# Diegotistical/OptionsLab

Hardware: AMD Instinct MI355X
Metric: MC path-steps/sec (1M paths × 252 steps Euro call); price vs BS |err|/σ (higher is better)
Workload: dtype f32 normals / f64 prices

## Files before the change

include/olmc.h:

```cpp
#ifndef OLMC_H
#define OLMC_H

#include <stdint.h>

#ifdef __cplusplus
extern "C" {
#endif

#define OLMC_ABI_VERSION 6

enum {
    OLMC_OK = 0,
    OLMC_ERR_ARG = 1,
    OLMC_ERR_HIP = 2,
    OLMC_ERR_STATE = 3,
    OLMC_ERR_RCCL = 4
};

enum { OLMC_STREAM_GBM = 0, OLMC_STREAM_HESTON = 1, OLMC_STREAM_JUMP = 2, OLMC_STREAM_KOU = 3 };
enum { OLMC_STREAM_HESTON_QE = 0x48514500 };
enum { OLMC_AVG_ARITHMETIC = 0, OLMC_AVG_GEOMETRIC = 1, OLMC_AVG_ARITHMETIC_FAST = 2 };
#define OLMC_MAX_BATCH 16

typedef struct olmc_stats {
// ... 139 lines not shown
                      const uint32_t* sv, const uint32_t* shift, int32_t bits, olmc_stats* out);
int olmc_european_qmc_cv(double S, double K, double T, double r, double sigma, double q, int is_call,
                         int64_t point_offset, int64_t n_paths, int32_t dims,
                         const uint32_t* sv, const uint32_t* shift, int32_t bits, olmc_cv_moments* out);

int olmc_european_qmc_batch(const olmc_option* opts, int32_t k, int64_t point_offset, int64_t n_paths, int32_t dims,
                            const uint32_t* sv, const uint32_t* shift, int32_t bits, olmc_stats* out );
int olmc_european_qmc_greeks_fd(double S, double K, double T, double r, double sigma, double q, int is_call,
                                int64_t n_paths, int32_t dims, const uint32_t* sv, const uint32_t* shift, int32_t bits,
                                int second_order, double* out9, olmc_stats* evals );

int olmc_european_qmc_terminal(double S, double T, double r, double sigma, double q,
                               int64_t point_offset, int64_t n_paths, int32_t dims,
                               const uint32_t* sv, const uint32_t* shift, int32_t bits,
                               int antithetic, double* out_host );

enum { OLMC_QMC_SEQUENTIAL = 0, OLMC_QMC_BRIDGE = 1 };
#define OLMC_QMC_BRIDGE_MAX_STEPS 1024
int olmc_asian_qmc(double S, double K, double T, double r, double sigma, double q, int is_call, int avg_kind, int construction,
                   int64_t point_offset, int64_t n_points, int32_t n_steps, const uint32_t* sv, const uint32_t* shift, int32_t bits,
                   int antithetic, olmc_stats* out);
int olmc_extrema_qmc(double S, double K, double T, double r, double sigma, double q, int is_call, int payoff, double barrier,
                     int construction, int64_t point_offset, int64_t n_points, int32_t n_steps, const uint32_t* sv,
                     const uint32_t* shift, int32_t bits, int antithetic, olmc_stats* out);
int olmc_asian_qmc_greeks_fd(double S, double K, double T, double r, double sigma, double q, int is_call, int avg_kind,
                             int construction, int64_t n_points, int32_t n_steps, const uint32_t* sv, const uint32_t* shift,
                             int32_t bits, int antithetic, int second_order, double* out9, olmc_stats* evals );
int olmc_extrema_qmc_greeks_fd(double S, double K, double T, double r, double sigma, double q, int is_call, int payoff, double barrier,
                               int construction, int64_t n_points, int32_t n_steps, const uint32_t* sv, const uint32_t* shift,
                               int32_t bits, int antithetic, int second_order, double* out9, olmc_stats* evals );

int olmc_autocallable_qmc(double S, double T, double r, double sigma, double q, double autocall_barrier, double coupon_barrier,
                          double coupon_rate, double ki_barrier, int32_t observation_freq, int construction,
                          int64_t point_offset, int64_t n_points, int32_t n_steps, const uint32_t* sv, const uint32_t* shift,
                          int32_t bits, int antithetic, olmc_stats* out);
int olmc_cliquet_qmc(double S, double T, double r, double sigma, double q, double local_cap, double local_floor, double global_cap,
                     double global_floor, int32_t n_periods, int construction, int64_t point_offset, int64_t n_points,
                     int32_t n_steps, const uint32_t* sv, const uint32_t* shift, int32_t bits, int antithetic, olmc_stats* out);

int olmc_american_lsm_qmc(double S, double K, double T, double r, double sigma, double q, int is_call, int construction,
                          int64_t n_points, int32_t n_steps, const uint32_t* sv, const uint32_t* shift, int32_t bits,
                          int32_t poly_degree, olmc_stats* out);
int olmc_exercise_boundary_qmc(double S, double K, double T, double r, double sigma, double q, int is_call, int construction,
                               int64_t n_points, int32_t n_steps, const uint32_t* sv, const uint32_t* shift, int32_t bits,
                               double* boundary_host);
int olmc_gbm_qmc_paths(double S, double T, double r, double sigma, double q, int construction, int64_t n_points, int32_t n_steps,
                       const uint32_t* sv, const uint32_t* shift, int32_t bits, int path_major, double* out_host);

int olmc_heston_qmc(double S, double K, double T, double r, double q, int is_call, double kappa, double theta, double sigma_v,
                    double rho, double v0, int construction, int64_t point_offset, int64_t n_points, int32_t n_steps,
                    const uint32_t* sv, const uint32_t* shift, int32_t bits, int antithetic, olmc_stats* out);
int olmc_heston_qmc_paths(double S, double T, double r, double q, double kappa, double theta, double sigma_v, double rho, double v0,
                          int construction, int64_t n_points, int32_t n_steps, const uint32_t* sv, const uint32_t* shift,
                          int32_t bits, int path_major, double* spot_host, double* var_host);

enum { OLMC_PATH_ASIAN_ARITHMETIC = 6, OLMC_PATH_ASIAN_GEOMETRIC = 7 };
int olmc_heston_path_payoff(double S, double K, double T, double r, double q, int is_call, double kappa, double theta, double sigma_v,
                            double rho, double v0, int payoff, double barrier, int64_t path_offset, int64_t n_local, int32_t n_steps,
                            uint64_t seed, int antithetic, olmc_stats* out);
int olmc_heston_qmc_path_payoff(double S, double K, double T, double r, double q, int is_call, double kappa, double theta, double sigma_v,
                                double rho, double v0, int payoff, double barrier, int construction, int64_t point_offset,
                                int64_t n_points, int32_t n_steps, const uint32_t* sv, const uint32_t* shift, int32_t bits,
                                int antithetic, olmc_stats* out);

int olmc_heston_surface(double S, double T, double r, double q, int is_call, double kappa, double theta, double sigma_v, double rho,
                        double v0, const double* strikes, const int32_t* steps, int32_t k, int64_t path_offset, int64_t n_local,
                        int32_t n_steps, uint64_t seed, int antithetic, olmc_stats* out );
int olmc_heston_qmc_surface(double S, double T, double r, double q, int is_call, double kappa, double theta, double sigma_v, double rho,
                            double v0, const double* strikes, const int32_t* steps, int32_t k, int construction, int64_t point_offset,
                            int64_t n_points, int32_t n_steps, const uint32_t* sv, const uint32_t* shift, int32_t bits, int antithetic,
                            olmc_stats* out );

typedef struct olmc_heston_scenario {
    double  S, K, T, r, q, kappa, theta, sigma_v, rho, v0;
    int32_t is_call;
    int32_t pad;
} olmc_heston_scenario;
#define OLMC_HESTON_MAX_RECURSIONS 6
int olmc_heston_scenario_layout(const olmc_heston_scenario* sc, int32_t k, int32_t* n_recursions, int32_t* group );
int olmc_heston_scenarios(const olmc_heston_scenario* sc, int32_t k, int64_t path_offset, int64_t n_local, int32_t n_steps, uint64_t seed,
                          int antithetic, olmc_stats* out );
int olmc_heston_qmc_scenarios(const olmc_heston_scenario* sc, int32_t k, int construction, int64_t point_offset, int64_t n_points,
                              int32_t n_steps, const uint32_t* sv, const uint32_t* shift, int32_t bits, int antithetic,
                              olmc_stats* out );
int olmc_heston_greeks_fd(double S, double K, double T, double r, double sigma, double q, int is_call, double kappa, double theta,
                          double sigma_v, double rho, int64_t n_paths, int32_t n_steps, uint64_t seed, int antithetic, int second_order,
                          double* out9, olmc_stats* evals );
int olmc_heston_qmc_greeks_fd(double S, double K, double T, double r, double sigma, double q, int is_call, double kappa, double theta,
                              double sigma_v, double rho, int construction, int64_t n_points, int32_t n_steps, const uint32_t* sv,
                              const uint32_t* shift, int32_t bits, int antithetic, int second_order, double* out9,
                              olmc_stats* evals );

int olmc_heston_qe_surface(double S, double T, double r, double q, int is_call, double kappa, double theta, double sigma_v, double rho,
                           double v0, const double* strikes, const int32_t* steps, int32_t k, int64_t path_offset, int64_t n_local,
                           int32_t n_steps, uint64_t seed, int antithetic, olmc_stats* out );
int olmc_heston_qe_qmc_surface(double S, double T, double r, double q, int is_call, double kappa, double theta, double sigma_v, double rho,
                               double v0, const double* strikes, const int32_t* steps, int32_t k, int construction, int64_t point_offset,
                               int64_t n_points, int32_t n_steps, const uint32_t* sv, const uint32_t* shift, int32_t bits, int antithetic,
                               olmc_stats* out );
int olmc_heston_qe_paths(double S, double T, double r, double q, double kappa, double theta, double sigma_v, double rho, double v0,
                         int64_t n_paths, int32_t n_steps, uint64_t seed, int path_major, double* spot_host, double* var_host);
int olmc_heston_qe_qmc_paths(double S, double T, double r, double q, double kappa, double theta, double sigma_v, double rho, double v0,
                             int construction, int64_t n_points, int32_t n_steps, const uint32_t* sv, const uint32_t* shift, int32_t bits,
                             int path_major, double* spot_host, double* var_host);

enum { OLMC_HESTON_EULER = 0, OLMC_HESTON_QE = 1 };
int olmc_heston_autocallable(double S, double T, double r, double q, double kappa, double theta, double sigma_v, double rho, double v0,
                             double autocall_barrier, double coupon_barrier, double coupon_rate, double ki_barrier, int32_t observation_freq,
                             int scheme, int64_t path_offset, int64_t n_local, int32_t n_steps, uint64_t seed, int antithetic,
                             olmc_stats* out);
int olmc_heston_autocallable_qmc(double S, double T, double r, double q, double kappa, double theta, double sigma_v, double rho, double v0,
                                 double autocall_barrier, double coupon_barrier, double coupon_rate, double ki_barrier,
                                 int32_t observation_freq, int scheme, int construction, int64_t point_offset, int64_t n_points,
                                 int32_t n_steps, const uint32_t* sv, const uint32_t* shift, int32_t bits, int antithetic, olmc_stats* out);
int olmc_heston_cliquet(double S, double T, double r, double q, double kappa, double theta, double sigma_v, double rho, double v0,
                        double local_cap, double local_floor, double global_cap, double global_floor, int32_t n_periods, int scheme,
                        int64_t path_offset, int64_t n_local, int32_t n_steps, uint64_t seed, int antithetic, olmc_stats* out);
int olmc_heston_cliquet_qmc(double S, double T, double r, double q, double kappa, double theta, double sigma_v, double rho, double v0,
                            double local_cap, double local_floor, double global_cap, double global_floor, int32_t n_periods, int scheme,
                            int construction, int64_t point_offset, int64_t n_points, int32_t n_steps, const uint32_t* sv,
                            const uint32_t* shift, int32_t bits, int antithetic, olmc_stats* out);

int olmc_multi_gpu_european(double S, double K, double T, double r, double sigma, double q, int is_call,
                            int64_t n_paths, int32_t n_steps, uint64_t seed, int antithetic,
                            int n_gpus, olmc_stats* out);
int olmc_multi_gpu_greeks_fd(double S, double K, double T, double r, double sigma, double q, int is_call,
                             int64_t n_paths, int32_t n_steps, uint64_t seed, int second_order,
                             int n_gpus, double* out9, olmc_stats* evals );
int olmc_multi_gpu_european_cv(double S, double K, double T, double r, double sigma, double q, int is_call,
                               int64_t n_paths, int32_t n_steps, uint64_t seed, int antithetic,
                               int n_gpus, olmc_cv_moments* out);
int olmc_multi_gpu_european_qmc(double S, double K, double T, double r, double sigma, double q, int is_call,
                                int64_t n_paths, int32_t dims, const uint32_t* sv, const uint32_t* shift, int32_t bits,
                                int n_gpus, olmc_stats* out);
int olmc_multi_gpu_european_qmc_greeks_fd(double S, double K, double T, double r, double sigma, double q, int is_call,
                                          int64_t n_paths, int32_t dims, const uint32_t* sv, const uint32_t* shift, int32_t bits,
                                          int second_order, int n_gpus, double* out9, olmc_stats* evals );
int olmc_multi_gpu_european_qmc_cv(double S, double K, double T, double r, double sigma, double q, int is_call,
                                   int64_t n_paths, int32_t dims, const uint32_t* sv, const uint32_t* shift, int32_t bits,
                                   int n_gpus, olmc_cv_moments* out);
int olmc_multi_gpu_spans(double* out8);

int olmc_fetch_dev(const double* d_src, int32_t n, void* hip_stream, double* out_host);

int olmc_combine_stats(const olmc_stats* parts, int32_t n_parts, double r, double T, olmc_stats* out);

int olmc_philox_words(uint64_t seed, int64_t path_offset, int64_t n_paths,
                      int32_t block0, int32_t n_blocks, uint32_t stream_tag, uint32_t* out_host);
int olmc_normals(uint64_t seed, int64_t path_offset, int64_t n_paths, int32_t n_steps,
                 float* out_host);

int olmc_profile_enable(int on);
enum { OLMC_TUNE_GRID_CAP = 2, OLMC_TUNE_QMC_BLOCK = 4, OLMC_TUNE_SPLIT_TAIL = 7, OLMC_TUNE_POLL = 8, OLMC_TUNE_SPLIT_SAT = 9,
       OLMC_TUNE_MULTI_LAUNCH = 10, OLMC_TUNE_STAGED_COPY = 11, OLMC_TUNE_PHILOX_TABLE = 12 };
int olmc_tune(int knob, int value);
int olmc_profile_reset(void);
int olmc_kernel_time(int64_t* launches, double* total_ms);

#ifdef __cplusplus
}
#endif
#endif
```

optionslab_amd/_hip.py:

```python
from __future__ import annotations

import ctypes as C
import importlib.util
import os
import sys
import threading
from typing import List, Optional, Sequence, Tuple

import numpy as np

from .exceptions import AccelerationError

LIBRARY_PATH = os.environ.get("OLMC_LIBRARY") or os.path.join(os.path.dirname(os.path.abspath(__file__)), "libolmc.so")
MAX_BATCH = 16
AVG_ARITHMETIC, AVG_GEOMETRIC, AVG_ARITHMETIC_FAST = 0, 1, 2
_U64 = (1 << 64) - 1


class Stats(C.Structure):
    _fields_ = [("sum", C.c_double), ("sumsq", C.c_double), ("n", C.c_int64),
                ("price", C.c_double), ("std_error", C.c_double)]


class Option(C.Structure):
# ... 864 lines not shown


def heston_qe_qmc_surface(S, T, r, q, is_call: bool, kappa, theta, sigma_v, rho, v0, strikes, steps, n_points: int, sv: np.ndarray,
                          shift: np.ndarray, bridge: bool = False, antithetic: bool = False, point_offset: int = 0) -> List[Stats]:
    sobol = _sobol_args(sv, shift, point_offset, n_points, 2)
    cells = _SurfaceCells(strikes, steps)
    return cells.answer(lib().olmc_heston_qe_qmc_surface(S, T, r, q, int(is_call), kappa, theta, sigma_v, rho, v0, *cells.run, _construction(bridge),
                                                         int(point_offset), int(n_points), *sobol.run, int(antithetic), cells.out))


HESTON_EULER, HESTON_QE = 0, 1


def _scheme(qe: bool) -> int:
    return HESTON_QE if qe else HESTON_EULER


def heston_autocallable(S, T, r, q, kappa, theta, sigma_v, rho, v0, autocall_barrier, coupon_barrier, coupon_rate, ki_barrier,
                        observation_freq: int, n_paths: int, n_steps: int, seed: int, antithetic: bool = False, path_offset: int = 0,
                        qe: bool = False) -> Stats:
    return _answer(lib().olmc_heston_autocallable(S, T, r, q, kappa, theta, sigma_v, rho, v0, autocall_barrier, coupon_barrier, coupon_rate, ki_barrier,
                                                  int(observation_freq), _scheme(qe), int(path_offset), int(n_paths), int(n_steps),
                                                  seed64(seed), int(antithetic), _byref(out := Stats())), out)


def heston_autocallable_qmc(S, T, r, q, kappa, theta, sigma_v, rho, v0, autocall_barrier, coupon_barrier, coupon_rate, ki_barrier,
                            observation_freq: int, n_points: int, sv: np.ndarray, shift: np.ndarray, bridge: bool = True,
                            antithetic: bool = False, point_offset: int = 0, qe: bool = False) -> Stats:
    sobol = _sobol_args(sv, shift, point_offset, n_points, 2)
    return _answer(lib().olmc_heston_autocallable_qmc(S, T, r, q, kappa, theta, sigma_v, rho, v0, autocall_barrier, coupon_barrier, coupon_rate, ki_barrier,
                                                      int(observation_freq), _scheme(qe), _construction(bridge), int(point_offset), int(n_points),
                                                      *sobol.run, int(antithetic), _byref(out := Stats())), out)


def heston_cliquet(S, T, r, q, kappa, theta, sigma_v, rho, v0, local_cap, local_floor, global_cap, global_floor, n_periods: int,
                   n_paths: int, n_steps: int, seed: int, antithetic: bool = False, path_offset: int = 0, qe: bool = False) -> Stats:
    return _answer(lib().olmc_heston_cliquet(S, T, r, q, kappa, theta, sigma_v, rho, v0, local_cap, local_floor, global_cap, global_floor, int(n_periods),
                                             _scheme(qe), int(path_offset), int(n_paths), int(n_steps),
                                             seed64(seed), int(antithetic), _byref(out := Stats())), out)


def heston_cliquet_qmc(S, T, r, q, kappa, theta, sigma_v, rho, v0, local_cap, local_floor, global_cap, global_floor, n_periods: int,
                       n_points: int, sv: np.ndarray, shift: np.ndarray, bridge: bool = True, antithetic: bool = False,
                       point_offset: int = 0, qe: bool = False) -> Stats:
    sobol = _sobol_args(sv, shift, point_offset, n_points, 2)
    return _answer(lib().olmc_heston_cliquet_qmc(S, T, r, q, kappa, theta, sigma_v, rho, v0, local_cap, local_floor, global_cap, global_floor, int(n_periods),
                                                 _scheme(qe), _construction(bridge), int(point_offset), int(n_points),
                                                 *sobol.run, int(antithetic), _byref(out := Stats())), out)


def heston_qe_paths(S, T, r, q, kappa, theta, sigma_v, rho, v0, n_paths: int, n_steps: int, seed: int, path_major: bool = False):
    return _spot_and_variance(lib().olmc_heston_qe_paths, n_paths, n_steps, path_major, S, T, r, q, kappa, theta, sigma_v, rho, v0,
                              int(n_paths), int(n_steps), seed64(seed))


def heston_qe_qmc_paths(S, T, r, q, kappa, theta, sigma_v, rho, v0, n_points: int, sv: np.ndarray, shift: np.ndarray, bridge: bool = False,
                        path_major: bool = False):
    sobol = _sobol_args(sv, shift, 0, n_points, 2)
    return _spot_and_variance(lib().olmc_heston_qe_qmc_paths, n_points, sobol.steps, path_major, S, T, r, q, kappa, theta, sigma_v, rho, v0,
                              _construction(bridge), int(n_points), *sobol.run)


def _basis(spot_basis: bool) -> int:
    return HA_BASIS_SPOT if spot_basis else HA_BASIS_SPOT_VARIANCE


def heston_american_lsm(S, K, T, r, q, is_call: bool, kappa, theta, sigma_v, rho, v0, n_paths: int, n_steps: int, seed: int, poly_degree: int = 2,
                        spot_basis: bool = False, qe: bool = False) -> Stats:
    return _answer(lib().olha_american_lsm(S, K, T, r, q, int(is_call), kappa, theta, sigma_v, rho, v0, _scheme(qe), _basis(spot_basis), int(poly_degree),
                                           int(n_paths), int(n_steps), seed64(seed), _byref(out := Stats())), out)


def heston_american_lsm_qmc(S, K, T, r, q, is_call: bool, kappa, theta, sigma_v, rho, v0, n_points: int, sv: np.ndarray, shift: np.ndarray,
                            bridge: bool = True, poly_degree: int = 2, spot_basis: bool = False, qe: bool = False) -> Stats:
    steps, psv, psh, bits = _sobol_args(sv, shift, 0, n_points, 2).run
    return _answer(lib().olha_american_lsm_qmc(S, K, T, r, q, int(is_call), kappa, theta, sigma_v, rho, v0, _scheme(qe), _basis(spot_basis), int(poly_degree),
                                               _construction(bridge), int(n_points), psv, psh, 2 * steps, bits, _byref(out := Stats())), out)


def heston_american_scales(S, K, T, r, q, is_call: bool, kappa, theta, sigma_v, v0, n_steps: int):
    out = [np.empty(int(n_steps) + 1 if n_steps >= 1 else 1, dtype=np.float64) for _ in range(4)]
    _check(load_library().olha_regressor_scales(S, K, T, r, q, int(is_call), kappa, theta, sigma_v, v0, int(n_steps), *[_dp(a) for a in out]))
    return tuple(out)


def multi_gpu_european(S, K, T, r, sigma, q, is_call: bool, n_paths: int, n_steps: int, seed: int, antithetic: bool,
                       n_gpus: int) -> Stats:
    return _answer(lib().olmc_multi_gpu_european(S, K, T, r, sigma, q, int(is_call), int(n_paths), int(n_steps), seed64(seed),
                                                 int(antithetic), int(n_gpus), _byref(out := Stats())), out)


def multi_gpu_greeks_fd(S, K, T, r, sigma, q, is_call: bool, n_paths: int, n_steps: int, seed: int, second_order: bool, n_gpus: int,
                        want_evals: bool = True) -> Tuple[List[float], List[Stats]]:
    return _greeks(want_evals, lib().olmc_multi_gpu_greeks_fd, S, K, T, r, sigma, q, int(is_call), int(n_paths), int(n_steps), seed64(seed),
                   int(second_order), int(n_gpus))


def multi_gpu_european_cv(S, K, T, r, sigma, q, is_call: bool, n_paths: int, n_steps: int, seed: int, antithetic: bool, n_gpus: int) -> CvMoments:
    return _answer(lib().olmc_multi_gpu_european_cv(S, K, T, r, sigma, q, int(is_call), int(n_paths), int(n_steps), seed64(seed),
                                                    int(antithetic), int(n_gpus), _byref(out := CvMoments())), out)


def multi_gpu_european_qmc(S, K, T, r, sigma, q, is_call: bool, n_paths: int, sv: np.ndarray, shift: np.ndarray, n_gpus: int) -> Stats:
    sobol = _sobol_args(sv, shift, 0, n_paths)
    return _answer(lib().olmc_multi_gpu_european_qmc(S, K, T, r, sigma, q, int(is_call), int(n_paths), *sobol.run, int(n_gpus), _byref(out := Stats())), out)


def multi_gpu_european_qmc_greeks_fd(S, K, T, r, sigma, q, is_call: bool, n_paths: int, sv: np.ndarray, shift: np.ndarray, second_order: bool,
                                     n_gpus: int, want_evals: bool = True) -> Tuple[List[float], List[Stats]]:
    sobol = _sobol_args(sv, shift, 0, n_paths)
    return _greeks(want_evals, lib().olmc_multi_gpu_european_qmc_greeks_fd, S, K, T, r, sigma, q, int(is_call), int(n_paths), *sobol.run,
                   int(second_order), int(n_gpus))


def multi_gpu_european_qmc_cv(S, K, T, r, sigma, q, is_call: bool, n_paths: int, sv: np.ndarray, shift: np.ndarray, n_gpus: int) -> CvMoments:
    sobol = _sobol_args(sv, shift, 0, n_paths)
    return _answer(lib().olmc_multi_gpu_european_qmc_cv(S, K, T, r, sigma, q, int(is_call), int(n_paths),
                                                        *sobol.run, int(n_gpus), _byref(out := CvMoments())), out)


def multi_gpu_spans() -> dict:
    out = (C.c_double * 8)()
    _check(lib().olmc_multi_gpu_spans(out))
    return dict(zip(("launch_us", "collective_us", "fetch_us", "drain_us", "total_us", "wake_us_max", "rank_launch_us_max", "rank_launch_us_min"), out))


def combine_stats(parts: Sequence[Tuple[float, float, int]], r: float, T: float) -> Stats:
    k = len(parts)
    arr = (Stats * k)(*[Stats(s, ss, int(n), 0.0, 0.0) for (s, ss, n) in parts])
    return _answer(load_library().olmc_combine_stats(arr, k, r, T, _byref(out := Stats())), out)


def philox_words(seed: int, path_offset: int, n_paths: int, block0: int, n_blocks: int, tag: int = 0) -> np.ndarray:
    out = np.empty((int(n_paths), int(n_blocks), 4), dtype=np.uint32)
    _check(lib().olmc_philox_words(seed64(seed), int(path_offset), int(n_paths), int(block0), int(n_blocks), int(tag),
                                   _pointer(out, C.c_uint32)))
    return out


def normals(seed: int, path_offset: int, n_paths: int, n_steps: int) -> np.ndarray:
    out = np.empty((int(n_paths), int(n_steps)), dtype=np.float32)
    _check(lib().olmc_normals(seed64(seed), int(path_offset), int(n_paths), int(n_steps), _pointer(out, C.c_float)))
    return out


TUNE_GRID_CAP = 2
TUNE_QMC_BLOCK = 4
TUNE_SPLIT_TAIL = 7
TUNE_POLL = 8
TUNE_SPLIT_SAT = 9
TUNE_MULTI_LAUNCH = 10
TUNE_STAGED_COPY = 11
TUNE_PHILOX_TABLE = 12


def tune(knob: int, value: int) -> None:
    _check(load_library().olmc_tune(int(knob), int(value)))


def profile_enable(on: bool) -> None:
    _check(lib().olmc_profile_enable(int(on)))


def profile_reset() -> None:
    _check(lib().olmc_profile_reset())


def kernel_time() -> Tuple[int, float]:
    n, ms = C.c_int64(0), C.c_double(0.0)
    _check(lib().olmc_kernel_time(C.byref(n), C.byref(ms)))
    return n.value, ms.value
```

optionslab_amd/csrc/olmc.hip:

```cpp
#include "olmc.h"
#include "olmc_local_vol.h"
#include "olmc_local_vol_qmc.h"
#include "olmc_jump.h"
#include "olha.h"
#include "olmc_kernels.h"
#include "olmc_local_vol_kernels.h"
#include "olmc_local_vol_qmc_kernels.h"
#include "olmc_jump_kernels.h"
#include "olmc_jump_scenario_kernels.h"
#include "olmc_heston_american_kernels.h"
#include "olmc_job_board.h"
#include "olmc_device_mem.h"

#include <dlfcn.h>
#include <sched.h>
#include <time.h>
#include <hip/hip_ext.h>
#include <rccl/rccl.h>

#include <algorithm>
#include <atomic>
#include <chrono>
#include <climits>
#include <condition_variable>
// ... 158 lines not shown
    DevicePool* pool = nullptr;
    CtxLease() = default;
    CtxLease(const CtxLease&) = delete;
    CtxLease& operator=(const CtxLease&) = delete;
    ~CtxLease() { release(); }
    void release() {
        if (!c) return;
        {
            std::lock_guard<std::mutex> lock(pool->mu);
            c->busy = false;
        }
        pool->idle.notify_all();
        c = nullptr;
    }
};

int ctx_lease_on(int dev, CtxLease* out) {
    DevicePool* pool = g_pool[dev].load(std::memory_order_acquire);
    if (!pool) return fail(OLMC_ERR_STATE, "device not initialised (call olmc_init)");
    HIP_TRY(hipSetDevice(dev));
    std::unique_lock<std::mutex> lock(pool->mu);
    for (;;) {
        for (DeviceCtx* c : pool->all)
            if (!c->busy) {
                c->busy = true;
                out->c = c;
                out->pool = pool;
                return OLMC_OK;
            }
        if (static_cast<int>(pool->all.size()) < kMaxContexts) {
            DeviceCtx* c = nullptr;
            const int rc = ctx_create(dev, &c);
            if (rc) return rc;
            c->busy = true;
            pool->all.push_back(c);
            out->c = c;
            out->pool = pool;
            return OLMC_OK;
        }
        pool->idle.wait(lock);
    }
}

int ctx_lease(CtxLease* out) {
    int dev = t_device >= 0 ? t_device : g_default_device.load(std::memory_order_acquire);
    if (dev < 0) {
        int rc = olmc_init(0);
        if (rc) return rc;
        dev = t_device;
    }
    return ctx_lease_on(dev, out);
}

int bulk_reserve(DeviceCtx* c, size_t bytes, Carver* spans = nullptr) {
    const int rc = c->bulk.reserve(bytes, [c] { return c->drain(); });
    if (spans) *spans = c->bulk.carve();
    return rc;
}

constexpr size_t kStageBytes = size_t(16) << 20, kStagedFrom = size_t(32) << 20;
int g_staged_copy = 0;

int copy_to_host(DeviceCtx* c, void* dst, const void* d_src, size_t bytes) {
    if (bytes < kStagedFrom || g_staged_copy < 0) {
        HIP_TRY(hipMemcpyAsync(dst, d_src, bytes, hipMemcpyDeviceToHost, c->stream));
        HIP_TRY(hipStreamSynchronize(c->stream));
        return OLMC_OK;
    }
    for (int i = 0; i < 2; ++i) {
        const int rc = c->stage[i].reserve(kStageBytes, no_users);
        if (rc) return rc;
        if (!c->stage_landed[i]) HIP_TRY(hipEventCreateWithFlags(&c->stage_landed[i], hipEventDisableTiming));
    }
    cpu_set_t cpus;
    int allowed = 4;
    if (sched_getaffinity(0, sizeof cpus, &cpus) == 0) allowed = CPU_COUNT(&cpus);
    const int n_threads = std::max(1, std::min(8, allowed / 2));
    const int64_t n_chunks = static_cast<int64_t>((bytes + kStageBytes - 1) / kStageBytes);
    std::atomic<int64_t> landed{0};
    std::atomic<int> copied[2] = {{0}, {0}};
    std::atomic<bool> give_up{false};
    auto chunk_len = [&](int64_t i) { return std::min(kStageBytes, bytes - static_cast<size_t>(i) * kStageBytes); };
    auto worker = [&](int w) {
        for (int64_t i = 0; i < n_chunks; ++i) {
            for (uint32_t spins = 0; landed.load(std::memory_order_acquire) <= i; ++spins) {
                if (give_up.load(std::memory_order_relaxed)) return;
                if ((spins & 0xFF) == 0xFF) sched_yield(); else __builtin_ia32_pause();
            }
            const size_t len = chunk_len(i), per = (len / n_threads + 4095) & ~size_t(4095);
            const size_t lo = std::min(len, per * w), hi = std::min(len, lo + per);
            if (hi > lo) std::memcpy(static_cast<char*>(dst) + static_cast<size_t>(i) * kStageBytes + lo, static_cast<const char*>(c->stage[i & 1].get()) + lo, hi - lo);
            copied[i & 1].fetch_add(1, std::memory_order_release);
        }
    };
    static const bool trace = std::getenv("OLMC_TRACE_COPY") != nullptr;
    using clock = std::chrono::steady_clock;
    auto us_since = [](clock::time_point t) { return std::chrono::duration<double, std::micro>(clock::now() - t).count(); };
    const auto t_begin = clock::now();
    double us_spawn = 0, us_first = 0, us_events = 0, us_workers = 0;
    std::vector<std::thread> threads;
    threads.reserve(n_threads);
    try {
        for (int w = 0; w < n_threads; ++w) threads.emplace_back(worker, w);
    } catch (const std::system_error&) {
        give_up.store(true);
        for (std::thread& t : threads) t.join();
        HIP_TRY(hipMemcpyAsync(dst, d_src, bytes, hipMemcpyDeviceToHost, c->stream));
        HIP_TRY(hipStreamSynchronize(c->stream));
        return OLMC_OK;
    }
    us_spawn = us_since(t_begin);
    hipError_t err = hipSuccess;
    for (int64_t i = 0; i < n_chunks && err == hipSuccess; ++i) {
        const int slot = static_cast<int>(i & 1);
        if (i >= 2) {
            const auto t = clock::now();
            for (uint32_t spins = 0; copied[slot].load(std::memory_order_acquire) < n_threads; ++spins)
                if ((spins & 0xFF) == 0xFF) sched_yield(); else __builtin_ia32_pause();
            copied[slot].store(0, std::memory_order_relaxed);
            us_workers += us_since(t);
        }
        err = hipMemcpyAsync(c->stage[slot].get(), static_cast<const char*>(d_src) + static_cast<size_t>(i) * kStageBytes, chunk_len(i), hipMemcpyDeviceToHost, c->stream);
        if (err == hipSuccess) err = hipEventRecord(c->stage_landed[slot], c->stream);
        if (err == hipSuccess && i >= 1) {
            const auto t = clock::now();
            err = hipEventSynchronize(c->stage_landed[slot ^ 1]);
            if (i == 1) us_first = us_since(t); else us_events += us_since(t);
            if (err == hipSuccess) landed.store(i, std::memory_order_release);
        }
    }
    {
        const auto t = clock::now();
        if (err == hipSuccess) err = hipEventSynchronize(c->stage_landed[(n_chunks - 1) & 1]);
        us_events += us_since(t);
    }
    if (err == hipSuccess) landed.store(n_chunks, std::memory_order_release);
    else give_up.store(true);
    const auto t_join = clock::now();
    for (std::thread& t : threads) t.join();
    if (trace)
        std::fprintf(stderr, "[olmc copy_to_host] %.1f MB, %lld chunks, %d threads: spawn %.0f us, first chunk landed (kernel + DMA) %.0f us, later event waits %.0f us, "
                             "waits for the copy threads %.0f us, last chunk out + join %.0f us, total %.0f us\n", bytes / 1e6, static_cast<long long>(n_chunks), n_threads,
                     us_spawn, us_first, us_events, us_workers, us_since(t_join), us_since(t_begin));
    if (err != hipSuccess) {
        (void)hipStreamSynchronize(c->stream);
        (void)hipGetLastError();
        return fail(OLMC_ERR_HIP, std::string("copy_to_host: ") + hipGetErrorString(err));
    }
    return OLMC_OK;
}

int g_multi_launch = 0;
int g_grid_cap = 0;
int g_qmc_block = 0;
int g_poll = 0;
int g_split_tail = 0;
int g_philox_table = 1;
int g_split_sat = 0;
#ifdef OLMC_WITH_PROBES
int g_fault_shard = 0;
int g_force_nv = 0;
int g_multi_rehearsal = 0;
int g_expect_table = 0;
std::atomic<int> g_expect_table_misses{0};
#endif

int32_t grid_for(int64_t n_paths, int32_t n_steps = INT32_MAX) { return path_grid(n_paths, n_steps, g_grid_cap); }

template <typename Kernel>
int resident_workgroups(Kernel kernel) {
    static std::mutex mu;
    static std::vector<std::pair<const void*, int>> cache;
    const void* key = reinterpret_cast<const void*>(kernel);
    std::lock_guard<std::mutex> lock(mu);
    for (const auto& e : cache)
        if (e.first == key) return e.second;
    int nb = 0;
    if (hipOccupancyMaxActiveBlocksPerMultiprocessor(&nb, kernel, kBlock, 0) != hipSuccess || nb < 1) {
        (void)hipGetLastError();
        nb = 1;
    }
    cache.emplace_back(key, nb);
    return nb;
}

int32_t european_launch_shape(const DeviceCtx* c, PathRange* pr, int occ, bool keep_grid = false) {
    pr->split_from = INT32_MAX;
    const int grid_cap = keep_grid ? 0 : g_grid_cap;
    const int32_t grid = path_grid(pr->count, pr->n_steps, grid_cap);
    const int64_t wgs = (pr->count + kBlock - 1) / kBlock;
    if (g_split_tail < 0 || grid_cap != 0 || wgs != grid) return grid;
    if ((pr->n_steps >> 2) / kGroup < 4 || c->cus < 1) return grid;
    int64_t per_cu = (pr->count / kBlock) / c->cus;
    if (occ >= 1 && g_split_sat > 0) {
        const int64_t r = per_cu % occ;
        if (r > 0 && r < std::min(g_split_sat, occ)) per_cu -= r;
    }
    const int64_t full = per_cu * c->cus;
    const int64_t rest = pr->count - full * kBlock;
    if (rest == 0) return grid;
    const int64_t split = (rest + kWave - 1) / kWave;
    if (full + split > kMaxGrid) return grid;
    pr->split_from = static_cast<int32_t>(full);
    return static_cast<int32_t>(full + split);
}

template <int NSETS, int MODE>
int european_occupancy(bool anti) {
    if (g_split_sat <= 0) return 0;
    return anti ? resident_workgroups(european_path_kernel<NSETS, true, MODE, false>) : resident_workgroups(european_path_kernel<NSETS, false, MODE, false>);
}

int make_ws(DeviceCtx* c, hipStream_t stream, int32_t grid, int nv, double* d_out, double tail, ReduceWs* ws) {
    const bool own = stream == c->stream;
    int idx = DeviceCtx::kSlots;
    if (!own) {
        idx = -1;
        for (int i = 0; i < DeviceCtx::kSlots && idx < 0; ++i)
            if (c->slots[i].claimed && !c->slots[i].shared && c->slots[i].owner == stream) idx = i;
        for (int i = 0; i < DeviceCtx::kSlots && idx < 0; ++i)
            if (!c->slots[i].claimed) { c->slots[i].claimed = true; c->slots[i].owner = stream; idx = i; }
        if (idx < 0) {
            idx = c->next_slot;
            c->next_slot = (c->next_slot + 1) % DeviceCtx::kSlots;
            DeviceCtx::WsSlot& taken = c->slots[idx];
            if (!taken.shared) {
                HIP_TRY(hipDeviceSynchronize());
                taken.shared = true;
                taken.used = false;
            }
        }
    }
    DeviceCtx::WsSlot& sl = c->slots[idx];
    c->cur_slot = idx;
    const bool guarded = !own && sl.shared;
    const size_t need = static_cast<size_t>(grid) * nv;
    int rc = sl.block_rows.reserve(sizeof(double) * need, [&] {
        if (!guarded) HIP_TRY(hipStreamSynchronize(stream));
        else if (sl.used) HIP_TRY(hipEventSynchronize(sl.done));
        return static_cast<int>(OLMC_OK);
    }, sizeof(double) << 16);
    if (rc) return rc;
    if (guarded && sl.used) HIP_TRY(hipStreamWaitEvent(stream, sl.done, 0));
    ws->block_rows = sl.block_rows.as<double>();
    ws->group_rows = sl.group_rows.as<double>();
    ws->counters = sl.counters.as<uint32_t>();
    ws->out = d_out;
    ws->tail = tail;
    ws->row_capacity = sl.block_rows.capacity() / sizeof(double);
#ifdef OLMC_WITH_PROBES
    if (g_force_nv > 0) ws->row_capacity = static_cast<uint64_t>(grid) * g_force_nv;
#endif
    ws->done_flag = nullptr;
    ws->done_value = 0;
    c->armed = 0;
    if (own && d_out == c->d_result && g_poll >= 0) {
        c->armed = ++c->seq;
        ws->done_flag = c->d_flag;
        ws->done_value = c->armed;
    }
    return OLMC_OK;
}

void ws_recover(DeviceCtx* c) {
    c->armed = 0;
    (void)hipDeviceSynchronize();
    (void)hipGetLastError();
    for (auto& sl : c->slots) (void)hipMemset(sl.counters.get(), 0, kCounterBytes);
}

void multi_recover(DeviceCtx* c) {
    c->armed = 0;
    (void)hipDeviceSynchronize();
    (void)hipGetLastError();
    if (c->multi.counters()) (void)hipMemset(c->multi.counters(), 0, c->multi.counter_bytes());
}

int after_launch(DeviceCtx* c, hipStream_t stream) {
    hipError_t e = hipGetLastError();
    if (e != hipSuccess) { ws_recover(c); return fail(OLMC_ERR_HIP, std::string("kernel launch: ") + hipGetErrorString(e)); }
    if (c->cur_slot == DeviceCtx::kSlots || !c->slots[c->cur_slot].shared) return OLMC_OK;
    DeviceCtx::WsSlot& sl = c->slots[c->cur_slot];
    HIP_TRY(hipEventRecord(sl.done, stream));
    sl.used = true;
    return OLMC_OK;
}

int prof_begin(DeviceCtx* c, hipStream_t s, EventPair* ep) {
    if (c->ev_free.empty()) {
        HIP_TRY(hipEventCreate(&ep->start));
        HIP_TRY(hipEventCreate(&ep->stop));
    } else {
        *ep = c->ev_free.back();
        c->ev_free.pop_back();
    }
    HIP_TRY(hipEventRecord(ep->start, s));
    return OLMC_OK;
}

int prof_acquire(DeviceCtx* c, EventPair* ep) {
    if (c->ev_free.empty()) {
        HIP_TRY(hipEventCreate(&ep->start));
        HIP_TRY(hipEventCreate(&ep->stop));
    } else {
        *ep = c->ev_free.back();
        c->ev_free.pop_back();
    }
    return OLMC_OK;
}

int prof_end(DeviceCtx* c, hipStream_t s, const EventPair& ep) {
    HIP_TRY(hipEventRecord(ep.stop, s));
    c->ev_pending.push_back(ep);
    return OLMC_OK;
}

int prof_drain(DeviceCtx* c) {
    for (const EventPair& ep : c->ev_pending) {
        float ms = 0.f;
        if (hipEventSynchronize(ep.stop) == hipSuccess && hipEventElapsedTime(&ms, ep.start, ep.stop) == hipSuccess) {
            c->prof_ms += ms;
            c->prof_launches += 1;
        } else {
            (void)hipGetLastError();
        }
        c->ev_free.push_back(ep);
    }
    c->ev_pending.clear();
    return OLMC_OK;
}


int check_paths(int64_t path_offset, int64_t n_local, int32_t n_steps) {
    if (n_local < 1) return fail(OLMC_ERR_ARG, "n_paths must be >= 1");
    if (n_steps < 1) return fail(OLMC_ERR_ARG, "n_steps must be >= 1");
    if (path_offset < 0) return fail(OLMC_ERR_ARG, "path_offset must be >= 0");
    return OLMC_OK;
}

PathRange make_range(int64_t path_offset, int64_t n_local, int32_t n_steps, uint64_t seed) {
    PathRange pr;
    pr.first = static_cast<uint64_t>(path_offset);
    pr.count = n_local;
    pr.n_steps = n_steps;
    pr.key0 = static_cast<uint32_t>(seed);
    pr.key1 = static_cast<uint32_t>(seed >> 32);
    pr.split_from = INT32_MAX;
    return pr;
}

template <typename Kernel, typename... Args>
void launch_timed(Kernel kernel, dim3 grid, dim3 block, hipStream_t s, const EventPair* timed, const Args&... args) {
    if (timed) hipExtLaunchKernelGGL(kernel, grid, block, 0, s, timed->start, timed->stop, 0, args...);
    else hipLaunchKernelGGL(kernel, grid, block, 0, s, args...);
}

template <typename F>
void with_bool(bool b, F&& f) {
    if (b) f(std::true_type{});
    else f(std::false_type{});
}

template <typename F>
void with_set_anti(int nsets, bool anti, F&& f) {
    with_bool(nsets == 8, [&](auto eight) { with_bool(anti, [&](auto a) { f(std::integral_constant<int, eight ? 8 : 16>{}, a); }); });
}

int prof_pair(DeviceCtx* c, EventPair* ep, const EventPair** timed) {
    *timed = nullptr;
    if (!g_profile) return OLMC_OK;
    int rc = prof_acquire(c, ep);
    if (rc) return rc;
    c->ev_pending.push_back(*ep);
    *timed = ep;
    return OLMC_OK;
}

PhiloxPrefix european_prefix(const PathRange& pr, bool strided) {
    PhiloxPrefix pp;
    const int32_t blocks = (pr.n_steps + 3) / 4;
    const uint64_t last = pr.first + static_cast<uint64_t>(pr.count) - 1;
    const bool table = g_philox_table != 0 && !strided && blocks <= kPrefixBlocks && (last >> 32) == (pr.first >> 32);
    philox_prefix(static_cast<uint64_t>(pr.key0) | static_cast<uint64_t>(pr.key1) << 32, static_cast<uint32_t>(pr.first >> 32), 0u, table ? blocks : 0, &pp);
    return pp;
}

template <int NSETS, int MODE>
void launch_european(bool anti, int32_t grid, hipStream_t s, const PathRange& pr, const ContractSet<NSETS>& cs,
                     const ReduceWs& ws, double* terminal, const EventPair* timed = nullptr) {
    const bool strided = static_cast<int64_t>(grid) * kBlock < pr.count;
    const PhiloxPrefix pp = european_prefix(pr, strided);
#ifdef OLMC_WITH_PROBES
    if (g_expect_table != 0 && (g_expect_table > 0) != (pp.n_blocks != 0)) g_expect_table_misses.fetch_add(1, std::memory_order_relaxed);
#endif
    auto launch = [&](auto strided_c, auto a) {
        launch_timed(european_path_kernel<NSETS, a, MODE, strided_c>, dim3(grid), dim3(kBlock), s, timed, pr, cs, ws, terminal, pp);
    };
    if constexpr (MODE == kSumOnly) with_bool(anti, [&](auto a) { launch(std::false_type{}, a); });
    else with_bool(strided, [&](auto strided_c) { with_bool(anti, [&](auto a) { launch(strided_c, a); }); });
}

int sync_or_recover(DeviceCtx* c, hipStream_t s);

template <typename Launch>
int launch_reduce(DeviceCtx* c, hipStream_t s, double* d_out, double tail, int nv, int32_t grid, Launch&& launch, bool profiled = true) {
    ReduceWs ws;
    int rc = make_ws(c, s, grid, nv, d_out, tail, &ws);
    if (rc) return rc;
    EventPair ep{};
    const EventPair* timed = nullptr;
    if (profiled) {
        rc = prof_pair(c, &ep, &timed);
        if (rc) return rc;
    }
    launch(grid, s, timed, ws);
    rc = after_launch(c, s);
    if (rc || d_out != c->d_result) return rc;
    return sync_or_recover(c, s);
}

void finish_one(const double* h, int64_t n, double r_disc, double T, bool bad, olmc_stats* out) {
    if (bad) nan_stats(n, out);
    else finish_stats(h[0], h[1], n, r_disc, T, out);
}

void finish_set(const double* h, const int* pos, int64_t n, const olmc_option* opts, int64_t k, bool extra_bad, bool lean, olmc_stats* st) {
    for (int64_t i = 0; i < k; ++i) {
        const int64_t slot = pos ? pos[i] : i;
        const olmc_option& o = opts[i];
        if (extra_bad || poisoned(o.S, o.K, o.T, o.r, o.sigma, o.q)) nan_stats(n, &st[i]);
        else if (lean) finish_stats(h[slot], std::nan(""), n, o.r, o.T, &st[i]);
        else finish_stats(h[2 * slot], h[2 * slot + 1], n, o.r, o.T, &st[i]);
    }
}

struct GbmStep {
    double dt, drift, vol;
};
GbmStep gbm_step(double T, int32_t n_steps, double r, double q, double sigma) {
    const double dt = T / n_steps;
    return {dt, (r - q - 0.5 * sigma * sigma) * dt, sigma * std::sqrt(dt)};
}

int run_batch_device(DeviceCtx* c, hipStream_t s, const olmc_option* opts, int32_t k, int64_t path_offset,
                     int64_t n_local, int32_t n_steps, uint64_t seed, int antithetic, double* d_out, double tail,
                     int* pos , bool profiled, bool* sums_only = nullptr
                     ,
                     bool keep_grid = false ) {
    PathRange pr = make_range(path_offset, n_local, n_steps, seed);
    const bool anti = antithetic != 0;
    const int nsets = k == 1 ? 1 : (k <= 8 ? 8 : 16);
    const int occ = nsets == 1 ? european_occupancy<1, kReduce>(anti) : (nsets == 8 ? european_occupancy<8, kReduce>(anti) : european_occupancy<16, kReduce>(anti));
    const int32_t grid = european_launch_shape(c, &pr, occ, keep_grid);
    const bool lean = sums_only && *sums_only && nsets > 1 && static_cast<int64_t>(grid) * kBlock >= n_local;
    if (sums_only) *sums_only = lean;
    return launch_reduce(c, s, d_out, tail, lean ? nsets : 2 * nsets, grid, [&](int32_t g, hipStream_t st, const EventPair* timed, const ReduceWs& ws) {
        auto fused = [&](auto width) {
            ContractSet<width> cs;
            group_contracts<width>(opts, k, n_steps, &cs, pos);
            if (!lean) launch_european<width, kReduce>(anti, g, st, pr, cs, ws, nullptr, timed);
            else launch_european<width, kSumOnly>(anti, g, st, pr, cs, ws, nullptr, timed);
        };
        if (nsets == 1) {
            ContractSet<1> cs;
            cs.c[0] = make_contract(opts[0], n_steps);
            cs.base_mask = 1u; cs.upper_continues_slot0 = 0;
            if (pos) pos[0] = 0;
            launch_european<1, kReduce>(anti, g, st, pr, cs, ws, nullptr, timed);
        } else if (nsets == 8) {
            fused(std::integral_constant<int, 8>{});
        } else {
            fused(std::integral_constant<int, 16>{});
        }
    }, profiled);
}

constexpr int64_t kSpinUs = 200, kYieldUs = 2000, kSleepUs = 20;

struct TimerSlack {
    long old = -1;
    void tighten() {
        if (old >= 0) return;
        old = prctl(PR_GET_TIMERSLACK, 0, 0, 0, 0);
        if (old >= 0 && prctl(PR_SET_TIMERSLACK, 1000UL, 0, 0, 0) != 0) old = -1;
    }
    ~TimerSlack() {
        if (old >= 0) (void)prctl(PR_SET_TIMERSLACK, static_cast<unsigned long>(old), 0, 0, 0);
    }
};

int wait_armed(DeviceCtx* c, hipStream_t s) {
    if (c->armed != 0) {
        const uint64_t want = c->armed;
        c->armed = 0;
        using clock = std::chrono::steady_clock;
        const auto t0 = clock::now();
        bool queried = false;
        int phase = 0;
        TimerSlack slack;
        for (uint32_t spins = 0;; ++spins) {
            if (__atomic_load_n(c->h_flag, __ATOMIC_ACQUIRE) == want) {
                if (queried) (void)hipGetLastError();
                return OLMC_OK;
            }
            if (phase == 0) {
                __builtin_ia32_pause();
                if ((spins & 0x3F) == 0x3F && clock::now() - t0 >= std::chrono::microseconds(kSpinUs)) phase = 1;
// ... 890 lines not shown
    CtxLease lease;
    rc = matrix_prologue(n_paths, n_steps, 2 * bytes, "path matrices would exceed 64 GB", &lease);
    if (rc) return rc;
    DeviceCtx* const c = lease.c;
    const auto hc = Scheme::make(S, T, r, q, 1, m, n_steps);
    const PathRange pr = make_range(0, n_paths, n_steps, seed);
    return heston_path_matrices(c, n_paths, n_steps, spot_host, var_host, [&](const EventPair* timed, double* d_spot, double* d_var) {
        with_bool(path_major != 0, [&](auto pm) {
            launch_timed(Scheme::template paths_kernel<decltype(pm)::value>(), dim3(grid_for(n_paths)), dim3(kBlock), c->stream, timed, pr, hc, S, d_spot,
                         d_var);
        });
    });
}
}

extern "C" int olmc_heston_paths(double S, double T, double r, double q, double kappa, double theta, double sigma_v, double rho,
                                 double v0, int64_t n_paths, int32_t n_steps, uint64_t seed, int path_major, double* spot_host,
                                 double* var_host) {
    return run_heston_paths<HestonEuler>(S, T, r, q, {kappa, theta, sigma_v, rho, v0}, n_paths, n_steps, seed, path_major, spot_host, var_host);
}

extern "C" int olmc_heston(double S, double K, double T, double r, double q, int is_call, double kappa, double theta,
                           double sigma_v, double rho, double v0, int64_t path_offset, int64_t n_local, int32_t n_steps,
                           uint64_t seed, int antithetic, olmc_stats* out) {
    if (!out) return fail(OLMC_ERR_ARG, "null pointer");
    const HestonModel m{kappa, theta, sigma_v, rho, v0};
    const int rc = heston_check(m);
    if (rc) return rc;
    const HestonContract hc = make_heston(S, K, T, r, q, is_call, m, n_steps);
    const bool bad = heston_poisoned(S, K, T, r, q, m);
    return run_structured(path_offset, n_local, n_steps, seed, antithetic, r, T, bad, out,
                          [&](int32_t grid, hipStream_t st, const EventPair* timed, const PathRange& pr, const ReduceWs& ws) {
                              with_bool(antithetic != 0, [&](auto a) { launch_timed(heston_kernel<a>, dim3(grid), dim3(kBlock), st, timed, pr, hc, ws); });
                          });
}

namespace {
int make_jump(double S, double K, double T, double r, double sigma, double q, int is_call, int model, double lambda_j,
              double a1, double a2, double a3, int32_t n_steps, JumpContract* out) {
    if (model != OLMC_JUMP_MERTON && model != OLMC_JUMP_KOU) return fail(OLMC_ERR_ARG, "bad jump model");
    if (!(lambda_j >= 0.0)) return fail(OLMC_ERR_ARG, "lambda_j must be non-negative");
    if (n_steps < 1) return fail(OLMC_ERR_ARG, "n_steps must be >= 1");
    JumpContract jc;
    const double dt = T / n_steps;
    double kappa;
    if (model == OLMC_JUMP_MERTON) {
        jc.mu_j = a1; jc.sigma_j = a2;
        jc.kou_p = 0.0; jc.inv_eta1 = 0.0; jc.inv_eta2 = 0.0;
        kappa = std::exp(a1 + 0.5 * a2 * a2) - 1;
    } else {
        jc.mu_j = 0.0; jc.sigma_j = 0.0;
        jc.kou_p = a1; jc.inv_eta1 = 1.0 / a2; jc.inv_eta2 = 1.0 / a3;
        kappa = a1 * a2 / (a2 - 1) + (1 - a1) * a3 / (a3 + 1) - 1;
    }
    jc.kou = model == OLMC_JUMP_KOU;
    jc.pad = 0;
    jc.log_s0 = std::log(S);
    jc.drift = (r - q - lambda_j * kappa - 0.5 * sigma * sigma) * dt;
    jc.vol = sigma * std::sqrt(dt);
    jc.strike = K;
    jc.sign = is_call ? 1.0 : -1.0;
    jc.lam_dt = lambda_j * dt;
    if (jc.lam_dt > 20.0) return fail(OLMC_ERR_ARG, "lambda_j * T / n_steps must be <= 20 jumps per step: raise n_steps");
    jc.p0 = std::exp(-jc.lam_dt);
    *out = jc;
    return OLMC_OK;
}
}

extern "C" int olmc_jump_diffusion(double S, double K, double T, double r, double sigma, double q, int is_call, int model,
                                   double lambda_j, double a1, double a2, double a3, int64_t path_offset, int64_t n_local,
                                   int32_t n_steps, uint64_t seed, olmc_stats* out) {
    JumpContract jc;
    int rc = make_jump(S, K, T, r, sigma, q, is_call, model, lambda_j, a1, a2, a3, n_steps, &jc);
    if (rc) return rc;
    const bool bad = poisoned(S, K, T, r, sigma, q) || std::isnan(lambda_j + a1 + a2 + a3);
    return run_structured(path_offset, n_local, n_steps, seed, 0, r, T, bad, out,
                          [&](int32_t grid, hipStream_t st, const EventPair* timed, const PathRange& pr, const ReduceWs& ws) {
                              launch_timed(jump_kernel, dim3(grid), dim3(kBlock), st, timed, pr, jc, ws);
                          });
}

extern "C" int olmc_jump_paths(double S, double T, double r, double sigma, double q, int model, double lambda_j, double a1,
                               double a2, double a3, int64_t n_paths, int32_t n_steps, uint64_t seed, int path_major,
                               double* out_host) {
    if (!out_host) return fail(OLMC_ERR_ARG, "null pointer");
    JumpContract jc;
    const int rc = make_jump(S, 0.0, T, r, sigma, q, 1, model, lambda_j, a1, a2, a3, n_steps, &jc);
    if (rc) return rc;
    return run_philox_matrix(n_paths, n_steps, seed, out_host, no_setup,
                             [&](DeviceCtx* c, int32_t grid, const PathRange& pr, double* d_paths) {
        with_bool(path_major != 0, [&](auto pm) {
            launch_timed(jump_paths_kernel<pm>, dim3(grid), dim3(kBlock), c->stream, nullptr, pr, jc, S, d_paths);
        });
    });
}

namespace {
struct SobolArgs {
    int construction;
    int64_t point_offset, n_points;
    int32_t n_steps;
    const uint32_t* sv;
    const uint32_t* shift;
    int32_t bits;
    int antithetic;
};

class SobolCall {
public:
    const bool bridge;
    const int64_t first, count;
    const int32_t n_steps, dims_per_step;
    const uint32_t* const sv;
    const uint32_t* const shift;
    const int32_t bits;
    const bool anti;

    static std::optional<SobolCall> make(const SobolArgs& a, int32_t dims_per_step, int* rc) {
        *rc = check(a, dims_per_step);
        if (*rc) return std::nullopt;
        return SobolCall(a.construction == OLMC_QMC_BRIDGE, a.point_offset, a.n_points, a.n_steps, dims_per_step, a.sv, a.shift, a.bits, a.antithetic != 0);
    }
    SobolCall over(int64_t lo, int64_t n) const { return SobolCall(bridge, lo, n, n_steps, dims_per_step, sv, shift, bits, anti); }

    int32_t dims() const { return n_steps * dims_per_step; }
    int64_t samples() const { return count * (anti ? 2 : 1); }
    QmcRange range() const { return QmcRange{static_cast<uint64_t>(first), count, n_steps, anti ? 1 : 0}; }

private:
    SobolCall(bool bridge_, int64_t first_, int64_t count_, int32_t n_steps_, int32_t dims_per_step_, const uint32_t* sv_, const uint32_t* shift_,
              int32_t bits_, bool anti_)
        : bridge(bridge_), first(first_), count(count_), n_steps(n_steps_), dims_per_step(dims_per_step_), sv(sv_), shift(shift_), bits(bits_),
          anti(anti_) {}

    static int check(const SobolArgs& a, int32_t dims_per_step) {
        if (a.construction != OLMC_QMC_SEQUENTIAL && a.construction != OLMC_QMC_BRIDGE) return fail(OLMC_ERR_ARG, "bad construction");
        if (a.construction == OLMC_QMC_BRIDGE && a.n_steps > OLMC_QMC_BRIDGE_MAX_STEPS)
            return fail(OLMC_ERR_ARG, "the Brownian-bridge construction takes at most OLMC_QMC_BRIDGE_MAX_STEPS (1024) dates");
        static_assert(OLMC_QMC_BRIDGE_MAX_STEPS == kQmcBridgeMaxSteps, "the header's cap is the kernel's LDS size");
        if (dims_per_step == 2 && (a.n_steps < 1 || a.n_steps > 10600))
            return fail(OLMC_ERR_ARG, "n_steps must be in [1, 10600]: a step takes two of the 21201 Sobol dimensions");
        const int32_t dims = a.n_steps * dims_per_step;
        if (!a.sv || !a.shift) return fail(OLMC_ERR_ARG, "null pointer");
        if (a.bits != kSobolBits) return fail(OLMC_ERR_ARG, "only 30-bit Sobol tables (SciPy's default) are supported");
        if (dims < 1 || dims > 21201) return fail(OLMC_ERR_ARG, "dims must be in [1, 21201]");
        const int rc = check_paths(a.point_offset, a.n_points, dims);
        if (rc) return rc;
        if (a.point_offset + a.n_points > (int64_t(1) << kSobolBits)) return fail(OLMC_ERR_ARG, "at most 2**30 Sobol points");
        return OLMC_OK;
    }
};

int qmc_table(DeviceCtx* c, const SobolCall& q, const uint32_t** d_sv, const uint32_t** d_shift) {
    const size_t sv_words = static_cast<size_t>(q.dims()) * kSobolBits;
    const int rc = c->sobol.put(q.sv, sizeof(uint32_t) * sv_words, q.shift, sizeof(uint32_t) * q.dims(), c->stream, [c] { return c->drain(); });
    if (rc) return rc;
    *d_sv = c->sobol.device<uint32_t>();
    *d_shift = *d_sv + sv_words;
    return OLMC_OK;
}

QmcShape qmc_shape(const SobolCall& q) {
    return qmc_launch_shape(q.first, q.count, q.dims(), g_qmc_block, g_grid_cap);
}

template <int MODE>
void launch_qmc_european(const QmcShape& sh, int32_t grid, hipStream_t s, const EventPair* timed, const QmcRange& qr, const Contract& ct,
                         const uint32_t* d_sv, const uint32_t* d_shift, const ReduceWs& ws, double* terminal) {
    auto go = [&](auto kernel) { launch_timed(kernel, dim3(grid), dim3(kBlock), s, timed, qr, ct, d_sv, d_shift, ws, terminal); };
    if (sh.blocks && sh.aligned8) go(european_qmc_block_kernel<MODE, true>);
    else if (sh.blocks) go(european_qmc_block_kernel<MODE, false>);
    else if (sh.split && sh.aligned) go(european_qmc_kernel<MODE, true, true>);
    else if (sh.split) go(european_qmc_kernel<MODE, true, false>);
    else go(european_qmc_kernel<MODE, false, false>);
}

template <int NSETS>
void launch_qmc_batch(const QmcShape& sh, int32_t grid, hipStream_t s, const EventPair* timed, const QmcRange& qr, const ContractSet<NSETS>& cs,
                      const uint32_t* d_sv, const uint32_t* d_shift, const ReduceWs& ws) {
    auto go = [&](auto kernel) { launch_timed(kernel, dim3(grid), dim3(kBlock), s, timed, qr, cs, d_sv, d_shift, ws); };
    if (sh.blocks && sh.aligned8) go(european_qmc_batch_kernel<NSETS, true, false, true>);
    else if (sh.blocks) go(european_qmc_batch_kernel<NSETS, true, false>);
    else if (sh.split && sh.aligned) go(european_qmc_batch_kernel<NSETS, false, true, true>);
    else if (sh.split) go(european_qmc_batch_kernel<NSETS, false, true>);
    else go(european_qmc_batch_kernel<NSETS, false, false>);
}

Contract qmc_contract(double S, double K, double T, double r, double sigma, double q, int is_call, int32_t dims, bool mirror) {
    const GbmStep g = gbm_step(T, dims, r, q, sigma);
    Contract ct;
    ct.vol = g.vol;
    ct.a = mirror ? std::log(S) + (r - q - 0.5 * sigma * sigma) * T : std::log(S) + g.drift * dims;
    ct.strike = K;
    ct.sign = is_call ? 1.0 : -1.0;
    ct.scale = 1.0;
    ct.neg_sign_strike = -ct.sign * K;
    ct.sign_scale = ct.sign;
    return ct;
}

int qmc_device(DeviceCtx* c, const Contract& ct, const SobolCall& q, bool five, double* d_out, double tail, bool profiled) {
    const uint32_t *d_sv, *d_shift;
    int rc = qmc_table(c, q, &d_sv, &d_shift);
    if (rc) return rc;
    const QmcRange qr = q.range();
    const QmcShape sh = qmc_shape(q);
    return launch_reduce(c, c->stream, d_out, tail, five ? 5 : 2, sh.grid, [&](int32_t grid, hipStream_t s, const EventPair* timed, const ReduceWs& ws) {
        if (five) launch_qmc_european<kControlVariate>(sh, grid, s, timed, qr, ct, d_sv, d_shift, ws, nullptr);
        else launch_qmc_european<kReduce>(sh, grid, s, timed, qr, ct, d_sv, d_shift, ws, nullptr);
    }, profiled);
}

int run_qmc(const olmc_option& o, const SobolCall& q, olmc_stats* out, double* terminal_host, olmc_cv_moments* cv = nullptr) {
    CtxLease lease;
    int rc = ctx_lease(&lease);
    if (rc) return rc;
    DeviceCtx* const c = lease.c;
    const Contract ct = qmc_contract(o.S, o.K, o.T, o.r, o.sigma, o.q, o.is_call, q.dims(), q.anti);
    if (!terminal_host) {
        rc = qmc_device(c, ct, q, cv != nullptr, c->d_result, -1.0, true);
        if (rc) return rc;
        if (cv) {
            cv_from_device(c->h_result, q.count, o.S, o.T, o.r, o.q, cv);
            if (poisoned(o.S, o.K, o.T, o.r, o.sigma, o.q)) cv->value = std::nan("");
            return OLMC_OK;
        }
        finish_one(c->h_result, q.count, o.r, o.T, poisoned(o.S, o.K, o.T, o.r, o.sigma, o.q), out);
        return OLMC_OK;
    }
    const size_t term_bytes = sizeof(double) * static_cast<size_t>(q.samples());
    Carver bulk;
    rc = bulk_reserve(c, term_bytes, &bulk);
    if (rc) return rc;
    const uint32_t *d_sv, *d_shift;
    rc = qmc_table(c, q, &d_sv, &d_shift);
    if (rc) return rc;
    double* d_term = bulk.take<double>(term_bytes / sizeof(double));
    const QmcShape sh = qmc_shape(q);
    launch_qmc_european<kTerminal>(sh, sh.grid, c->stream, nullptr, q.range(), ct, d_sv, d_shift, ReduceWs{}, d_term);
    HIP_TRY(hipGetLastError());
    c->armed = 0;
    return copy_to_host(c, terminal_host, d_term, term_bytes);
}

int run_qmc_checked(const olmc_option& o, const SobolArgs& a, olmc_stats* out, double* terminal_host, olmc_cv_moments* cv = nullptr) {
    int rc;
    const auto q = SobolCall::make(a, 1, &rc);
    return q ? run_qmc(o, *q, out, terminal_host, cv) : rc;
}
}

extern "C" int olmc_european_qmc_cv(double S, double K, double T, double r, double sigma, double q, int is_call,
                                    int64_t point_offset, int64_t n_paths, int32_t dims, const uint32_t* sv,
                                    const uint32_t* shift, int32_t bits, olmc_cv_moments* out) {
    if (!out) return fail(OLMC_ERR_ARG, "null pointer");
    return run_qmc_checked(make_option(S, K, T, r, sigma, q, is_call), {OLMC_QMC_SEQUENTIAL, point_offset, n_paths, dims, sv, shift, bits, 0}, nullptr,
                           nullptr, out);
}

extern "C" int olmc_european_qmc(double S, double K, double T, double r, double sigma, double q, int is_call,
                                 int64_t point_offset, int64_t n_paths, int32_t dims, const uint32_t* sv,
                                 const uint32_t* shift, int32_t bits, olmc_stats* out) {
    if (!out) return fail(OLMC_ERR_ARG, "null pointer");
    return run_qmc_checked(make_option(S, K, T, r, sigma, q, is_call), {OLMC_QMC_SEQUENTIAL, point_offset, n_paths, dims, sv, shift, bits, 0}, out,
                           nullptr);
}

extern "C" int olmc_european_qmc_terminal(double S, double T, double r, double sigma, double q, int64_t point_offset,
                                          int64_t n_paths, int32_t dims, const uint32_t* sv, const uint32_t* shift,
                                          int32_t bits, int antithetic, double* out_host) {
    if (!out_host) return fail(OLMC_ERR_ARG, "null pointer");
    return run_qmc_checked(make_option(S, 0.0, T, r, sigma, q, 1), {OLMC_QMC_SEQUENTIAL, point_offset, n_paths, dims, sv, shift, bits, antithetic},
                           nullptr, out_host);
}

namespace {
int qmc_bridge_plan(DeviceCtx* c, int32_t n, QmcBridgePlan* plan) {
    const size_t ab_bytes = (sizeof(uint32_t) * static_cast<size_t>(n) + 7) & ~size_t(7), bytes = ab_bytes + sizeof(double) * 3 * n;
    const int rc = c->bridge.ensure(n, bytes, c->stream, [c] { return c->drain(); }, [&](unsigned char* host) {
        uint32_t* ab = reinterpret_cast<uint32_t*>(host);
        double* coef = reinterpret_cast<double*>(host + ab_bytes);
        std::vector<std::pair<int32_t, int32_t>> queue{{0, n}};
        int32_t k = 1;
        for (size_t head = 0; head < queue.size(); ++head) {
            const int32_t a = queue[head].first, b = queue[head].second;
            if (b - a < 2) continue;
            const int32_t m = (a + b) / 2;
            if (k >= n) return fail(OLMC_ERR_ARG, "bridge plan overflow");
            ab[k] = static_cast<uint32_t>(a) | (static_cast<uint32_t>(b) << 16);
            coef[k] = static_cast<double>(b - m) / (b - a);
            coef[n + k] = static_cast<double>(m - a) / (b - a);
            coef[2 * n + k] = std::sqrt(static_cast<double>((m - a) * (b - m)) / (b - a));
            ++k;
            queue.emplace_back(a, m);
            queue.emplace_back(m, b);
        }
        if (k != n) return fail(OLMC_ERR_ARG, "bridge plan is incomplete");
        return static_cast<int>(OLMC_OK);
    });
    if (rc) return rc;
    plan->ab = c->bridge.device<uint32_t>();
    plan->coef = reinterpret_cast<const double*>(c->bridge.device<unsigned char>() + ab_bytes);
    return OLMC_OK;
}

struct QmcPathLaunch {
    const uint32_t* d_sv;
    const uint32_t* d_shift;
    QmcBridgePlan plan;
    QmcRange qr;
    int32_t grid;
    bool bridge, anti;
    double inv_steps;
    double* slabs = nullptr;
};
int qmc_path_setup(DeviceCtx* c, const SobolCall& q, QmcPathLaunch* pl) {
    int rc = qmc_table(c, q, &pl->d_sv, &pl->d_shift);
    if (rc) return rc;
    pl->plan = QmcBridgePlan{nullptr, nullptr};
    pl->bridge = q.bridge;
    if (pl->bridge) {
        rc = qmc_bridge_plan(c, q.n_steps, &pl->plan);
        if (rc) return rc;
    }
    pl->qr = q.range();
    pl->grid = qmc_point_grid(q.count, g_grid_cap);
    pl->anti = q.anti;
    pl->inv_steps = 1.0 / q.n_steps;
    return OLMC_OK;
}

template <typename F>
void with_bridge_anti(const QmcPathLaunch& pl, F&& f) {
    with_bool(pl.bridge, [&](auto b) { with_bool(pl.anti, [&](auto a) { f(b, a); }); });
}

template <typename F>
void with_qmc_path_family(int family, F&& f) {
    if (family == kQmcAsianArithmetic) f(std::integral_constant<int, kQmcAsianArithmetic>{});
    else if (family == kQmcAsianGeometric) f(std::integral_constant<int, kQmcAsianGeometric>{});
    else f(std::integral_constant<int, kQmcExtrema>{});
}

template <typename Shape, typename Launch, typename Finish>
int run_qmc_reduce(const SobolCall& q, int nv, Shape shape, Launch launch, Finish finish) {
    CtxLease lease;
    int rc = ctx_lease(&lease);
    if (rc) return rc;
    DeviceCtx* const c = lease.c;
    QmcPathLaunch pl;
    rc = qmc_path_setup(c, q, &pl);
    if (rc) return rc;
    rc = shape(c, q, &pl);
    if (rc) return rc;
    rc = launch_reduce(c, c->stream, c->d_result, -1.0, nv, pl.grid,
                       [&](int32_t g, hipStream_t s, const EventPair* timed, const ReduceWs& ws) { launch(g, s, timed, pl, ws); });
    if (rc) return rc;
    finish(c->h_result, q.samples());
    return OLMC_OK;
}
inline int qmc_point_shape(DeviceCtx*, const SobolCall&, QmcPathLaunch*) { return OLMC_OK; }
auto qmc_stats(double r_for_discount, double T, bool poisoned_inputs, olmc_stats* out) {
    return [=](const double* h, int64_t n) { finish_one(h, n, r_for_discount, T, poisoned_inputs, out); };
}

int run_qmc_path(int family, int payoff, const olmc_option& o, double barrier, const SobolArgs& args, olmc_stats* out) {
    if (!out) return fail(OLMC_ERR_ARG, "null pointer");
    int rc;
    const auto q = SobolCall::make(args, 1, &rc);
    if (!q) return rc;
    const ExtremaContract ec = make_extrema(o.S, o.K, o.T, o.r, o.sigma, o.q, o.is_call, family == kQmcExtrema ? payoff : 0, barrier, q->n_steps);
    const bool bad = poisoned(o.S, o.K, o.T, o.r, o.sigma, o.q) || std::isnan(barrier);
    return run_qmc_reduce(*q, 2, qmc_point_shape, [&](int32_t g, hipStream_t s, const EventPair* timed, const QmcPathLaunch& pl, const ReduceWs& ws) {
        with_qmc_path_family(family, [&](auto f) {
            with_bridge_anti(pl, [&](auto b, auto a) {
                launch_timed(qmc_path_kernel<f, b, a>, dim3(g), dim3(kBlock), s, timed, pl.qr, ec, pl.inv_steps, pl.d_sv, pl.d_shift, pl.plan, ws);
            });
        });
    }, qmc_stats(o.r, o.T, bad, out));
}

int run_qmc_path_greeks(int family, int payoff, const olmc_option& o, double barrier, const SobolArgs& args, int second_order, double* out9,
                        olmc_stats* evals) {
    if (!out9) return fail(OLMC_ERR_ARG, "null pointer");
    if (!(o.T > 0.0)) return fail(OLMC_ERR_ARG, "T must be > 0");
    int rc;
    const auto q = SobolCall::make(args, 1, &rc);
    if (!q) return rc;
    const GreeksSet gs(o.S, o.K, o.T, o.r, o.sigma, o.q, o.is_call, second_order);
    ExtremaGreeksSet es;
    if (const char* bad = extrema_greeks_layout(gs, q->n_steps, payoff, barrier, o.K, o.is_call, &es, 1.0)) return fail(OLMC_ERR_STATE, bad);
    const int nsets = gs.nsets();
    return run_qmc_reduce(*q, 2 * nsets, qmc_point_shape, [&](int32_t g, hipStream_t s, const EventPair* timed, const QmcPathLaunch& pl, const ReduceWs& ws) {
        with_qmc_path_family(family, [&](auto f) {
            with_bool(pl.bridge, [&](auto b) {
                with_set_anti(nsets, pl.anti, [&](auto width, auto a) {
                    launch_timed(qmc_path_greeks_kernel<f, b, a, width>, dim3(g), dim3(kBlock), s, timed, pl.qr, es, pl.inv_steps, pl.d_sv, pl.d_shift,
                                 pl.plan, ws);
                });
            });
        });
    }, [&](const double* h, int64_t n) {
        olmc_stats st[OLMC_MAX_BATCH];
        finish_set(h, nullptr, n, gs.o, gs.k, false, false, st);
        gs.finish(st, o.T, out9, evals);
    });
}
}

extern "C" int olmc_asian_qmc(double S, double K, double T, double r, double sigma, double q, int is_call, int avg_kind, int construction,
                              int64_t point_offset, int64_t n_points, int32_t n_steps, const uint32_t* sv, const uint32_t* shift, int32_t bits,
                              int antithetic, olmc_stats* out) {
    if (avg_kind != OLMC_AVG_ARITHMETIC && avg_kind != OLMC_AVG_GEOMETRIC) return fail(OLMC_ERR_ARG, "bad avg_kind (arithmetic or geometric)");
    return run_qmc_path(avg_kind == OLMC_AVG_GEOMETRIC ? kQmcAsianGeometric : kQmcAsianArithmetic, 0, make_option(S, K, T, r, sigma, q, is_call), 0.0,
                        {construction, point_offset, n_points, n_steps, sv, shift, bits, antithetic}, out);
}

extern "C" int olmc_extrema_qmc(double S, double K, double T, double r, double sigma, double q, int is_call, int payoff, double barrier,
                                int construction, int64_t point_offset, int64_t n_points, int32_t n_steps, const uint32_t* sv,
                                const uint32_t* shift, int32_t bits, int antithetic, olmc_stats* out) {
    if (payoff < OLMC_BARRIER_UP_OUT || payoff > OLMC_LOOKBACK_FIXED) return fail(OLMC_ERR_ARG, "bad payoff");
    if (payoff <= OLMC_BARRIER_DOWN_IN && !(barrier > 0.0)) return fail(OLMC_ERR_ARG, "Barrier must be positive");
    return run_qmc_path(kQmcExtrema, payoff, make_option(S, K, T, r, sigma, q, is_call), payoff <= OLMC_BARRIER_DOWN_IN ? barrier : 0.0,
                        {construction, point_offset, n_points, n_steps, sv, shift, bits, antithetic}, out);
}

extern "C" int olmc_asian_qmc_greeks_fd(double S, double K, double T, double r, double sigma, double q, int is_call, int avg_kind,
                                        int construction, int64_t n_points, int32_t n_steps, const uint32_t* sv, const uint32_t* shift,
                                        int32_t bits, int antithetic, int second_order, double* out9, olmc_stats* evals) {
    if (avg_kind != OLMC_AVG_ARITHMETIC && avg_kind != OLMC_AVG_GEOMETRIC)
        return fail(OLMC_ERR_ARG, "bad avg_kind (arithmetic or geometric: the fp32-exponent form has no Sobol path)");
    return run_qmc_path_greeks(avg_kind == OLMC_AVG_GEOMETRIC ? kQmcAsianGeometric : kQmcAsianArithmetic, 0, make_option(S, K, T, r, sigma, q, is_call),
                               0.0, {construction, 0, n_points, n_steps, sv, shift, bits, antithetic}, second_order, out9, evals);
}

extern "C" int olmc_extrema_qmc_greeks_fd(double S, double K, double T, double r, double sigma, double q, int is_call, int payoff, double barrier,
                                          int construction, int64_t n_points, int32_t n_steps, const uint32_t* sv, const uint32_t* shift,
                                          int32_t bits, int antithetic, int second_order, double* out9, olmc_stats* evals) {
    if (payoff < OLMC_BARRIER_UP_OUT || payoff > OLMC_LOOKBACK_FIXED) return fail(OLMC_ERR_ARG, "bad payoff");
    if (payoff <= OLMC_BARRIER_DOWN_IN && !(barrier > 0.0)) return fail(OLMC_ERR_ARG, "Barrier must be positive");
    return run_qmc_path_greeks(kQmcExtrema, payoff, make_option(S, K, T, r, sigma, q, is_call), payoff <= OLMC_BARRIER_DOWN_IN ? barrier : 0.0,
                               {construction, 0, n_points, n_steps, sv, shift, bits, antithetic}, second_order, out9, evals);
}

namespace {
uint32_t qmc_date_magic(int32_t d) { return static_cast<uint32_t>((uint64_t(1) << 31) / static_cast<uint64_t>(d)) + 1u; }
}

extern "C" int olmc_autocallable_qmc(double S, double T, double r, double sigma, double q, double autocall_barrier, double coupon_barrier,
                                     double coupon_rate, double ki_barrier, int32_t observation_freq, int construction,
                                     int64_t point_offset, int64_t n_points, int32_t n_steps, const uint32_t* sv, const uint32_t* shift,
                                     int32_t bits, int antithetic, olmc_stats* out) {
    if (!out) return fail(OLMC_ERR_ARG, "null pointer");
    int rc;
    const auto call = SobolCall::make({construction, point_offset, n_points, n_steps, sv, shift, bits, antithetic}, 1, &rc);
    if (!call) return rc;
    rc = autocall_check(observation_freq, n_steps);
    if (rc) return rc;
    const AutocallSetup a = make_autocall(S, T, r, sigma, q, autocall_barrier, coupon_barrier, coupon_rate, ki_barrier, observation_freq, n_steps);
    const uint32_t magic = qmc_date_magic(observation_freq);
    return run_qmc_reduce(*call, 2, qmc_point_shape, [&](int32_t g, hipStream_t s, const EventPair* timed, const QmcPathLaunch& pl, const ReduceWs& ws) {
        with_bridge_anti(pl, [&](auto b, auto m) {
            launch_timed(qmc_autocall_kernel<b, m>, dim3(g), dim3(kBlock), s, timed, pl.qr, a.ac, a.obs_rate, magic, pl.d_sv, pl.d_shift, pl.plan, ws);
        });
    }, qmc_stats(0.0, T, a.bad, out));
}

extern "C" int olmc_cliquet_qmc(double S, double T, double r, double sigma, double q, double local_cap, double local_floor, double global_cap,
                                double global_floor, int32_t n_periods, int construction, int64_t point_offset, int64_t n_points,
                                int32_t n_steps, const uint32_t* sv, const uint32_t* shift, int32_t bits, int antithetic, olmc_stats* out) {
    if (!out) return fail(OLMC_ERR_ARG, "null pointer");
    int rc;
    const auto call = SobolCall::make({construction, point_offset, n_points, n_steps, sv, shift, bits, antithetic}, 1, &rc);
    if (!call) return rc;
    rc = cliquet_check(n_periods, n_steps);
    if (rc) return rc;
    const CliquetContract cc = make_cliquet(S, T, r, sigma, q, local_cap, local_floor, global_cap, global_floor, n_periods, n_steps);
    const uint32_t magic = qmc_date_magic(cc.steps_per_period);
    const bool bad = cliquet_poisoned(S, T, r, sigma, q, local_cap, local_floor, global_cap, global_floor);
    return run_qmc_reduce(*call, 2, qmc_point_shape, [&](int32_t g, hipStream_t s, const EventPair* timed, const QmcPathLaunch& pl, const ReduceWs& ws) {
        with_bridge_anti(pl, [&](auto b, auto m) {
            launch_timed(qmc_cliquet_kernel<b, m>, dim3(g), dim3(kBlock), s, timed, pl.qr, cc, magic, pl.d_sv, pl.d_shift, pl.plan, ws);
        });
    }, qmc_stats(r, T, bad, out));
}

namespace {
int qmc_matrix_prologue(const SobolCall& q, double bytes, CtxLease* lease, bool reserve = true) {
    return matrix_prologue(q.count, q.n_steps, bytes, "path matrix would exceed 64 GB: lower n_paths or n_steps", lease, reserve);
}

int32_t qmc_block_grid(const SobolCall& q) { return qmc_blocks_grid((q.first + q.count - 1) / kWave - q.first / kWave + 1, g_grid_cap); }

int qmc_matrix_setup(DeviceCtx* c, const SobolCall& q, QmcPathLaunch* pl) {
    const int rc = qmc_path_setup(c, q, pl);
    pl->grid = qmc_block_grid(q);
    return rc;
}

int qmc_matrix(DeviceCtx* c, const SobolCall& q, const LsmContract& lc, bool path_major, double* d_paths) {
    QmcPathLaunch pl;
    const int rc = qmc_matrix_setup(c, q, &pl);
    if (rc) return rc;
    with_bool(pl.bridge, [&](auto b) {
        with_bool(path_major, [&](auto pm) {
            launch_timed(lsm_qmc_paths_kernel<b, pm>, dim3(pl.grid), dim3(kBlock), c->stream, nullptr, pl.qr, lc, pl.d_sv, pl.d_shift, pl.plan, d_paths);
        });
    });
    HIP_TRY(hipGetLastError());
    return OLMC_OK;
}
}

extern "C" int olmc_american_lsm_qmc(double S, double K, double T, double r, double sigma, double q, int is_call, int construction,
                                     int64_t n_points, int32_t n_steps, const uint32_t* sv, const uint32_t* shift, int32_t bits,
                                     int32_t poly_degree, olmc_stats* out) {
    if (!out) return fail(OLMC_ERR_ARG, "null pointer");
    if (poly_degree < 1 || poly_degree > kLsmMaxDegree) return fail(OLMC_ERR_ARG, "poly_degree must be in [1, 4]");
    int rc;
    const auto call = SobolCall::make({construction, 0, n_points, n_steps, sv, shift, bits, 0}, 1, &rc);
    if (!call) return rc;
    CtxLease lease;
    rc = qmc_matrix_prologue(*call, lsm_bytes(n_points, n_steps), &lease);
    if (rc) return rc;
    DeviceCtx* const c = lease.c;
    Carver bulk = c->bulk.carve();
    double* d_paths = bulk.take<double>((static_cast<size_t>(n_steps) + 1) * n_points);
    const LsmContract lc = lsm_contract(S, K, T, r, sigma, q, is_call, n_steps, poly_degree);
    EventPair ep{};
    if (g_profile) { rc = prof_begin(c, c->stream, &ep); if (rc) return rc; }
    rc = qmc_matrix(c, *call, lc, false, d_paths);
    if (rc) return rc;
    rc = lsm_chain(c, S, K, T, r, sigma, q, is_call, lc, n_points, n_steps, d_paths, &bulk);
    if (rc) return rc;
    if (g_profile) { rc = prof_end(c, c->stream, ep); if (rc) return rc; }
    finish_one(c->h_result, n_points, 0.0, T, poisoned(S, K, T, r, sigma, q), out);
    return OLMC_OK;
}

extern "C" int olmc_exercise_boundary_qmc(double S, double K, double T, double r, double sigma, double q, int is_call, int construction,
                                          int64_t n_points, int32_t n_steps, const uint32_t* sv, const uint32_t* shift, int32_t bits,
                                          double* boundary_host) {
    if (!boundary_host) return fail(OLMC_ERR_ARG, "null pointer");
    const size_t rows = static_cast<size_t>(n_steps) + 1;
    const double bytes = 8.0 * static_cast<double>(n_points) * (n_steps + 1.0);
    int rc;
    const auto call = SobolCall::make({construction, 0, n_points, n_steps, sv, shift, bits, 0}, 1, &rc);
    if (!call) return rc;
    CtxLease lease;
    rc = qmc_matrix_prologue(*call, bytes, &lease, false);
    if (rc) return rc;
    DeviceCtx* const c = lease.c;
    const size_t path_bytes = (static_cast<size_t>(bytes) + 255) / 256 * 256;
    Carver bulk;
    rc = bulk_reserve(c, path_bytes + rows * sizeof(double), &bulk);
    if (rc) return rc;
    double* d_paths = bulk.take<double>(path_bytes / sizeof(double));
    double* d_boundary = bulk.take<double>(rows);
    rc = qmc_matrix(c, *call, lsm_contract(S, K, T, r, sigma, q, is_call, n_steps, 1), false, d_paths);
    if (rc) return rc;
    hipLaunchKernelGGL(exercise_boundary_kernel, dim3(static_cast<uint32_t>(rows)), dim3(kBoundaryThreads), 0, c->stream, d_paths, n_points, K,
                       is_call ? 1.0 : -1.0, (is_call ? 90.0 : 10.0) / 100.0, d_boundary);
    HIP_TRY(hipGetLastError());
    HIP_TRY(hipMemcpyAsync(boundary_host, d_boundary, rows * sizeof(double), hipMemcpyDeviceToHost, c->stream));
    HIP_TRY(hipStreamSynchronize(c->stream));
    return OLMC_OK;
}

extern "C" int olmc_gbm_qmc_paths(double S, double T, double r, double sigma, double q, int construction, int64_t n_points, int32_t n_steps,
                                  const uint32_t* sv, const uint32_t* shift, int32_t bits, int path_major, double* out_host) {
    if (!out_host) return fail(OLMC_ERR_ARG, "null pointer");
    const double bytes = 8.0 * static_cast<double>(n_points) * (n_steps + 1.0);
    int rc;
    const auto call = SobolCall::make({construction, 0, n_points, n_steps, sv, shift, bits, 0}, 1, &rc);
    if (!call) return rc;
    CtxLease lease;
    rc = qmc_matrix_prologue(*call, bytes, &lease);
    if (rc) return rc;
    DeviceCtx* const c = lease.c;
    LsmContract lc = lsm_contract(S, S, T, r, sigma, q, 0, n_steps, 1);
    lc.s_first = S;
    rc = qmc_matrix(c, *call, lc, path_major != 0, c->bulk.as<double>());
    if (rc) return rc;
    return copy_to_host(c, out_host, c->bulk.get(), static_cast<size_t>(bytes));
}

namespace {
int heston_slabs(DeviceCtx* c, int32_t n_steps, int32_t* grid, int32_t factors = 2) {
    const HestonSlabs hs = heston_slab_shape(n_steps, *grid, c->cus, factors);
    *grid = hs.grid;
    return c->heston_w.reserve(hs.bytes, [c] { return c->drain(); });
}

int heston_qmc_shape(DeviceCtx* c, const SobolCall& q, QmcPathLaunch* pl) {
    pl->grid = qmc_block_grid(q);
    pl->slabs = nullptr;
    if (!pl->bridge) return OLMC_OK;
    const int rc = heston_slabs(c, q.n_steps, &pl->grid, q.dims_per_step);
    pl->slabs = c->heston_w.as<double>();
    return rc;
}

template <typename Scheme>
int run_heston_qmc_paths(double S, double T, double r, double q, const HestonModel& m, const SobolArgs& args, int path_major, double* spot_host,
                         double* var_host) {
    if (!spot_host || !var_host) return fail(OLMC_ERR_ARG, "null pointer");
    int rc = heston_qmc_scheme_check<Scheme>(m, args.construction);
    if (rc) return rc;
    const auto call = SobolCall::make(args, 2, &rc);
    if (!call) return rc;
    const double bytes = 8.0 * static_cast<double>(call->count) * (call->n_steps + 1.0);
    CtxLease lease;
    rc = qmc_matrix_prologue(*call, 2 * bytes, &lease);
    if (rc) return rc;
    DeviceCtx* const c = lease.c;
    const auto hc = Scheme::make(S, T, r, q, 1, m, call->n_steps);
    QmcPathLaunch pl;
    rc = qmc_matrix_setup(c, *call, &pl);
    if (rc) return rc;
    return heston_path_matrices(c, call->count, call->n_steps, spot_host, var_host, [&](const EventPair* timed, double* d_spot, double* d_var) {
        with_bool(path_major != 0, [&](auto pm) {
            if constexpr (Scheme::kBridge) {
                with_bool(pl.bridge, [&](auto b) {
                    launch_timed(heston_qmc_paths_kernel<b, pm>, dim3(pl.grid), dim3(kBlock), c->stream, timed, pl.qr, hc, S, pl.d_sv, pl.d_shift, pl.plan,
                                 d_spot, d_var);
                });
            } else {
                launch_timed(heston_qe_qmc_paths_kernel<pm>, dim3(pl.grid), dim3(kBlock), c->stream, timed, pl.qr, hc, S, pl.d_sv, pl.d_shift, d_spot, d_var);
            }
        });
    });
}
}

extern "C" int olmc_heston_qmc(double S, double K, double T, double r, double q, int is_call, double kappa, double theta, double sigma_v,
// ... 1531 lines not shown
        return run_batch_device(c, c->stream, &o, 1, lo, n_local, n_steps, seed, antithetic, d_send, n, nullptr, false);
    }, host);
    if (rc) return rc;
    finish_one(host, static_cast<int64_t>(host[2]), r, T, poisoned(S, K, T, r, sigma, q), out);
    return OLMC_OK;
}

extern "C" int olmc_multi_gpu_greeks_fd(double S, double K, double T, double r, double sigma, double q, int is_call,
                                        int64_t n_paths, int32_t n_steps, uint64_t seed, int second_order, int n_gpus,
                                        double* out9, olmc_stats* evals) {
    if (!out9) return fail(OLMC_ERR_ARG, "null pointer");
    if (!(T > 0.0)) return fail(OLMC_ERR_ARG, "T must be > 0 (price() returns intrinsic value without simulating)");
    const GreeksSet gs(S, K, T, r, sigma, q, is_call, second_order);
    const int nsets = gs.k <= 8 ? 8 : 16;
    int pos[OLMC_MAX_BATCH] = {};
    double host[kMultiValues] = {};
    const int rc = multi_gpu_run(n_gpus, n_paths, n_steps, 2 * nsets + 1, [&](int rank, int64_t lo, int64_t n_local, DeviceCtx* c, double* d_send) {
        int other[OLMC_MAX_BATCH];
        return run_batch_device(c, c->stream, gs.o, gs.k, lo, n_local, n_steps, seed, 1, d_send, static_cast<double>(2 * n_local),
                                rank == 0 ? pos : other, false);
    }, host);
    if (rc) return rc;
    olmc_stats st[OLMC_MAX_BATCH];
    finish_set(host, pos, static_cast<int64_t>(host[2 * nsets]), gs.o, gs.k, false, false, st);
    gs.finish(st, T, out9, evals);
    return OLMC_OK;
}

extern "C" int olmc_multi_gpu_european_cv(double S, double K, double T, double r, double sigma, double q, int is_call,
                                          int64_t n_paths, int32_t n_steps, uint64_t seed, int antithetic, int n_gpus,
                                          olmc_cv_moments* out) {
    if (!out) return fail(OLMC_ERR_ARG, "null pointer");
    const olmc_option o = make_option(S, K, T, r, sigma, q, is_call);
    double host[6] = {};
    const int rc = multi_gpu_run(n_gpus, n_paths, n_steps, 6, [&](int, int64_t lo, int64_t n_local, DeviceCtx* c, double* d_send) {
        return cv_device(c, c->stream, o, lo, n_local, n_steps, seed, antithetic, d_send, static_cast<double>(n_local * (antithetic ? 2 : 1)), false);
    }, host);
    if (rc) return rc;
    cv_from_device(host, static_cast<int64_t>(host[5]), S, T, r, q, out);
    if (poisoned(S, K, T, r, sigma, q)) out->value = std::nan("");
    return OLMC_OK;
}

extern "C" int olmc_multi_gpu_european_qmc(double S, double K, double T, double r, double sigma, double q, int is_call,
                                           int64_t n_paths, int32_t dims, const uint32_t* sv, const uint32_t* shift, int32_t bits,
                                           int n_gpus, olmc_stats* out) {
    if (!out) return fail(OLMC_ERR_ARG, "null pointer");
    int rc;
    const auto call = SobolCall::make({OLMC_QMC_SEQUENTIAL, 0, n_paths, dims, sv, shift, bits, 0}, 1, &rc);
    if (!call) return rc;
    const Contract ct = qmc_contract(S, K, T, r, sigma, q, is_call, dims, false);
    double host[3] = {0, 0, 0};
    rc = multi_gpu_run(n_gpus, n_paths, dims, 3, [&](int, int64_t lo, int64_t n_local, DeviceCtx* c, double* d_send) {
        return qmc_device(c, ct, call->over(lo, n_local), false, d_send, static_cast<double>(n_local), false);
    }, host, true);
    if (rc) return rc;
    finish_one(host, static_cast<int64_t>(host[2]), r, T, poisoned(S, K, T, r, sigma, q), out);
    return OLMC_OK;
}

extern "C" int olmc_multi_gpu_european_qmc_greeks_fd(double S, double K, double T, double r, double sigma, double q, int is_call,
                                                     int64_t n_paths, int32_t dims, const uint32_t* sv, const uint32_t* shift,
                                                     int32_t bits, int second_order, int n_gpus, double* out9, olmc_stats* evals) {
    if (!out9) return fail(OLMC_ERR_ARG, "null pointer");
    if (!(T > 0.0)) return fail(OLMC_ERR_ARG, "T must be > 0 (price() returns intrinsic value without simulating)");
    int rc;
    const auto call = SobolCall::make({OLMC_QMC_SEQUENTIAL, 0, n_paths, dims, sv, shift, bits, 0}, 1, &rc);
    if (!call) return rc;
    const GreeksSet gs(S, K, T, r, sigma, q, is_call, second_order);
    const int nsets = gs.k <= 8 ? 8 : 16;
    int pos[OLMC_MAX_BATCH] = {};
    double host[kMultiValues] = {};
    rc = multi_gpu_run(n_gpus, n_paths, dims, 2 * nsets + 1, [&](int rank, int64_t lo, int64_t n_local, DeviceCtx* c, double* d_send) {
        int other[OLMC_MAX_BATCH];
        return qmc_batch_device(c, gs.o, gs.k, call->over(lo, n_local), d_send, static_cast<double>(n_local), rank == 0 ? pos : other, false);
    }, host, true);
    if (rc) return rc;
    olmc_stats st[OLMC_MAX_BATCH];
    finish_set(host, pos, static_cast<int64_t>(host[2 * nsets]), gs.o, gs.k, false, false, st);
    gs.finish(st, T, out9, evals);
    return OLMC_OK;
}

extern "C" int olmc_multi_gpu_european_qmc_cv(double S, double K, double T, double r, double sigma, double q, int is_call,
                                              int64_t n_paths, int32_t dims, const uint32_t* sv, const uint32_t* shift, int32_t bits,
                                              int n_gpus, olmc_cv_moments* out) {
    if (!out) return fail(OLMC_ERR_ARG, "null pointer");
    int rc;
    const auto call = SobolCall::make({OLMC_QMC_SEQUENTIAL, 0, n_paths, dims, sv, shift, bits, 0}, 1, &rc);
    if (!call) return rc;
    const Contract ct = qmc_contract(S, K, T, r, sigma, q, is_call, dims, false);
    double host[6] = {};
    rc = multi_gpu_run(n_gpus, n_paths, dims, 6, [&](int, int64_t lo, int64_t n_local, DeviceCtx* c, double* d_send) {
        return qmc_device(c, ct, call->over(lo, n_local), true, d_send, static_cast<double>(n_local), false);
    }, host, true);
    if (rc) return rc;
    cv_from_device(host, static_cast<int64_t>(host[5]), S, T, r, q, out);
    if (poisoned(S, K, T, r, sigma, q)) out->value = std::nan("");
    return OLMC_OK;
}

extern "C" int olmc_multi_gpu_spans(double* out8) {
    if (!out8) return fail(OLMC_ERR_ARG, "null pointer");
    for (int i = 0; i < 8; ++i) out8[i] = t_multi_spans[i];
    return OLMC_OK;
}

extern "C" int olmc_philox_words(uint64_t seed, int64_t path_offset, int64_t n_paths, int32_t block0, int32_t n_blocks,
                                 uint32_t stream_tag, uint32_t* out_host) {
    if (!out_host || n_paths < 1 || n_blocks < 1 || block0 < 0 || path_offset < 0) return fail(OLMC_ERR_ARG, "bad arguments");
    CtxLease lease;
    int rc = ctx_lease(&lease);
    if (rc) return rc;
    DeviceCtx* const c = lease.c;
    const size_t bytes = sizeof(uint32_t) * 4 * static_cast<size_t>(n_paths) * n_blocks;
    Carver bulk;
    rc = bulk_reserve(c, bytes, &bulk);
    if (rc) return rc;
    uint32_t* d_words = bulk.take<uint32_t>(bytes / sizeof(uint32_t));
    const int64_t total = n_paths * n_blocks;
    const int grid = static_cast<int>(std::min<int64_t>((total + 255) / 256, 4096));
    hipLaunchKernelGGL(philox_words_kernel, dim3(grid), dim3(256), 0, c->stream, static_cast<uint64_t>(path_offset), n_paths,
                       block0, n_blocks, stream_tag, static_cast<uint32_t>(seed), static_cast<uint32_t>(seed >> 32), d_words);
    HIP_TRY(hipGetLastError());
    HIP_TRY(hipMemcpyAsync(out_host, d_words, bytes, hipMemcpyDeviceToHost, c->stream));
    HIP_TRY(hipStreamSynchronize(c->stream));
    return OLMC_OK;
}

extern "C" int olmc_normals(uint64_t seed, int64_t path_offset, int64_t n_paths, int32_t n_steps, float* out_host) {
    if (!out_host || n_paths < 1 || n_steps < 1 || path_offset < 0) return fail(OLMC_ERR_ARG, "bad arguments");
    CtxLease lease;
    int rc = ctx_lease(&lease);
    if (rc) return rc;
    DeviceCtx* const c = lease.c;
    const size_t bytes = sizeof(float) * static_cast<size_t>(n_paths) * n_steps;
    Carver bulk;
    rc = bulk_reserve(c, bytes, &bulk);
    if (rc) return rc;
    float* d_z = bulk.take<float>(bytes / sizeof(float));
    const int64_t total = n_paths * ((n_steps + 3) / 4);
    const int grid = static_cast<int>(std::min<int64_t>((total + 255) / 256, 4096));
    hipLaunchKernelGGL(normals_kernel, dim3(grid), dim3(256), 0, c->stream, static_cast<uint64_t>(path_offset), n_paths,
                       n_steps, static_cast<uint32_t>(seed), static_cast<uint32_t>(seed >> 32), d_z);
    HIP_TRY(hipGetLastError());
    HIP_TRY(hipMemcpyAsync(out_host, d_z, bytes, hipMemcpyDeviceToHost, c->stream));
    HIP_TRY(hipStreamSynchronize(c->stream));
    return OLMC_OK;
}

extern "C" int olmc_tune(int knob, int value) {
    if (knob == OLMC_TUNE_GRID_CAP && value >= 0) { g_grid_cap = value; return OLMC_OK; }
    if (knob == OLMC_TUNE_QMC_BLOCK && value >= -1 && value <= 2) { g_qmc_block = value; return OLMC_OK; }
    if (knob == OLMC_TUNE_POLL && value >= -1 && value <= 0) { g_poll = value; return OLMC_OK; }
    if (knob == OLMC_TUNE_SPLIT_TAIL && value >= -1 && value <= 0) { g_split_tail = value; return OLMC_OK; }
    if (knob == OLMC_TUNE_SPLIT_SAT && value >= 0 && value <= 16) { g_split_sat = value; return OLMC_OK; }
    if (knob == OLMC_TUNE_MULTI_LAUNCH && value >= -1 && value <= 0) { g_multi_launch = value; return OLMC_OK; }
    if (knob == OLMC_TUNE_STAGED_COPY && value >= -1 && value <= 0) { g_staged_copy = value; return OLMC_OK; }
    if (knob == OLMC_TUNE_PHILOX_TABLE && value >= 0 && value <= 1) { g_philox_table = value; return OLMC_OK; }
    return fail(OLMC_ERR_ARG, "unknown tuning knob or value");
}

namespace {
template <typename Fn>
int with_all_contexts(Fn fn) {
    int dev = t_device >= 0 ? t_device : g_default_device.load(std::memory_order_acquire);
    if (dev < 0) {
        int rc = olmc_init(0);
        if (rc) return rc;
        dev = t_device;
    }
    DevicePool* pool = g_pool[dev].load(std::memory_order_acquire);
    if (!pool) return fail(OLMC_ERR_STATE, "device not initialised (call olmc_init)");
    HIP_TRY(hipSetDevice(dev));
    std::vector<DeviceCtx*> mine;
    {
        std::unique_lock<std::mutex> lock(pool->mu);
        pool->idle.wait(lock, [&] { return std::none_of(pool->all.begin(), pool->all.end(), [](const DeviceCtx* c) { return c->busy; }); });
        mine = pool->all;
        for (DeviceCtx* c : mine) c->busy = true;
    }
    int rc = OLMC_OK;
    for (DeviceCtx* c : mine) {
        const int r = fn(c);
        if (r && !rc) rc = r;
    }
    {
        std::lock_guard<std::mutex> lock(pool->mu);
        for (DeviceCtx* c : mine) c->busy = false;
    }
    pool->idle.notify_all();
    return rc;
}
}

extern "C" int olmc_profile_enable(int on) {
    g_profile = on != 0;
    if (g_profile && (t_device >= 0 || g_default_device.load() >= 0)) {
        CtxLease lease;
        int rc = ctx_lease(&lease);
        if (rc) return rc;
        DeviceCtx* const c = lease.c;
        constexpr size_t kPool = 4096;
        while (c->ev_free.size() + c->ev_pending.size() < kPool) {
            EventPair ep{};
            HIP_TRY(hipEventCreate(&ep.start));
            HIP_TRY(hipEventCreate(&ep.stop));
            c->ev_free.push_back(ep);
        }
    }
    return OLMC_OK;
}

extern "C" int olmc_profile_reset(void) {
    return with_all_contexts([](DeviceCtx* c) {
        const int rc = prof_drain(c);
        c->prof_launches = 0;
        c->prof_ms = 0.0;
        return rc;
    });
}

extern "C" int olmc_kernel_time(int64_t* launches, double* total_ms) {
    if (!launches || !total_ms) return fail(OLMC_ERR_ARG, "null pointer");
    int64_t n = 0;
    double ms = 0.0;
    const int rc = with_all_contexts([&](DeviceCtx* c) {
        const int r = prof_drain(c);
        n += c->prof_launches;
        ms += c->prof_ms;
        return r;
    });
    if (rc) return rc;
    *launches = n;
    *total_ms = ms;
    return OLMC_OK;
}
```

optionslab_amd/csrc/olmc_device_mem.h:

```cpp
#ifndef OLMC_DEVICE_MEM_H
#define OLMC_DEVICE_MEM_H

#include <algorithm>
#include <cassert>
#include <cstddef>
#include <cstdint>
#include <cstring>
#include <utility>
#include <vector>

namespace olmc {

inline size_t grown(size_t need, size_t have, size_t floor, size_t factor) { return std::max(need, std::max(floor, factor * have)); }

class Carver {
    char* base_;
    size_t size_, off_ = 0;
public:
    Carver(void* base = nullptr, size_t size = 0) : base_(static_cast<char*>(base)), size_(size) {}
    template <typename T>
    T* take(size_t n) {
        off_ = (off_ + alignof(T) - 1) / alignof(T) * alignof(T);
        assert(off_ + n * sizeof(T) <= size_);
        T* p = reinterpret_cast<T*>(base_ + off_);
        off_ += n * sizeof(T);
        return p;
    }
};

template <class B, bool PINNED>
class Block {
    void* p_ = nullptr;
    void* alias_ = nullptr;
    size_t cap_ = 0;
public:
    Block() = default;
    Block(Block&& o) noexcept { swap(o); }
    Block& operator=(Block&& o) noexcept { Block t(std::move(o)); swap(t); return *this; }
    Block(const Block&) = delete;
    Block& operator=(const Block&) = delete;
    ~Block() { (void)reset(); }
    void swap(Block& o) noexcept { std::swap(p_, o.p_); std::swap(alias_, o.alias_); std::swap(cap_, o.cap_); }

    void* get() const { return p_; }
    size_t capacity() const { return cap_; }
    template <typename T> T* as() const { return static_cast<T*>(p_); }
    template <typename T> T* alias() const { return static_cast<T*>(alias_); }
    Carver carve() const { return Carver(p_, cap_); }

    int reset() {
        void* p = p_;
        p_ = alias_ = nullptr;
        cap_ = 0;
        if (!p) return 0;
        return PINNED ? B::free_pinned(p) : B::free(p);
    }

    template <typename Quiesce>
    int reserve(size_t bytes, Quiesce&& quiesce, size_t floor = 0, size_t factor = 0, bool mapped = false) {
        if (bytes <= cap_) return 0;
        const size_t cap = grown(bytes, cap_, floor, factor);
        if (p_) {
            int e = quiesce();
            if (e) return e;
            e = reset();
            if (e) return e;
        }
        void* p = nullptr;
        int e = PINNED ? B::alloc_pinned(&p, cap, mapped) : B::alloc(&p, cap);
        if (e) return e;
        if (PINNED && mapped) {
            e = B::device_alias(&alias_, p);
            if (e) { alias_ = nullptr; (void)B::free_pinned(p); return e; }
        }
        p_ = p;
        cap_ = cap;
        return 0;
    }
};
template <class B> using DeviceBlock = Block<B, false>;
template <class B> using PinnedBlock = Block<B, true>;

template <class B>
class CachedUpload {
    DeviceBlock<B> dev_;
    std::vector<unsigned char> mirror_;
    int64_t key_ = 0;
    bool valid_ = false;

    template <typename Quiesce, typename Fill>
    int refill(size_t bytes, typename B::Stream s, Quiesce&& quiesce, Fill&& fill, size_t floor = 0) {
        valid_ = false;
        mirror_.resize(bytes);
        int e = fill(mirror_.data());
        if (!e) e = dev_.reserve(bytes, quiesce, floor);
        if (!e) e = B::upload(dev_.get(), mirror_.data(), bytes, s);
        valid_ = e == 0;
        return e;
    }
public:
    template <typename T> const T* device() const { return dev_.template as<const T>(); }

    template <typename Quiesce>
    int put(const void* a, size_t na, const void* b, size_t nb, typename B::Stream s, Quiesce&& quiesce) {
        if (valid_ && mirror_.size() == na + nb && std::memcmp(mirror_.data(), a, na) == 0 && std::memcmp(mirror_.data() + na, b, nb) == 0) return 0;
        return refill(na + nb, s, quiesce, [&](unsigned char* m) { std::memcpy(m, a, na); std::memcpy(m + na, b, nb); return 0; });
    }
    template <typename Quiesce, typename Build>
    int ensure(int64_t key, size_t bytes, typename B::Stream s, Quiesce&& quiesce, Build&& build) {
        if (valid_ && key_ == key && mirror_.size() == bytes) return 0;
        valid_ = false;
        key_ = key;
        if (const int e = dev_.get() ? quiesce() : 0) return e;
        return refill(bytes, s, quiesce, [&](unsigned char* m) { std::memset(m, 0, bytes); return build(m); });
    }
    template <typename Quiesce, typename Fill>
    int upload(size_t bytes, typename B::Stream s, Quiesce&& quiesce, Fill&& fill, size_t floor = 0) { return refill(bytes, s, quiesce, fill, floor); }
};

template <class B, class Opt, size_t COUNTER_STRIDE>
class BatchWorkspace {
    DeviceBlock<B> dev_;
    PinnedBlock<B> host_;
    size_t cap_ = 0, bpo_ = 0;
    size_t off_done_ = 0, off_opts_ = 0, off_rows_ = 0, hoff_out_ = 0;
    static size_t align(size_t b) { return (b + 255) / 256 * 256; }
public:
    struct Views {
        uint32_t *d_cnt, *d_done;
        Opt* d_opts;
        double* d_rows;
        Opt* h_opts;
        const double* h_out;
        double* d_out;
    };
    size_t capacity() const { return cap_; }
    size_t rows_per_contract() const { return bpo_; }
    void* counters() const { return cap_ ? dev_.get() : nullptr; }
    size_t counter_bytes() const { return off_opts_; }

    int reserve(size_t n_options, size_t bpo, typename B::Stream s, Views* v) {
        if (n_options > cap_ || bpo > bpo_) {
            const size_t cap = n_options > cap_ ? grown(n_options, cap_, 64, 2) : cap_, bpo_cap = std::max(bpo, bpo_);
            const size_t b_cnt = align(sizeof(uint32_t) * cap * COUNTER_STRIDE), b_done = 256, b_opts = align(sizeof(Opt) * cap);
            const size_t b_rows = align(sizeof(double) * 2 * bpo_cap * cap);
            cap_ = bpo_ = 0;
            bool waited = false;
            auto quiesce = [&] { const int e = waited ? 0 : B::wait(s); waited = true; return e; };
            int e = dev_.reserve(b_cnt + b_done + b_opts + b_rows, quiesce);
            if (!e) e = host_.reserve(b_opts + align(sizeof(double) * 2 * cap), quiesce, 0, 0, true);
            if (!e) e = B::zero(dev_.get(), b_cnt + b_done, s);
            if (e) return e;
            off_done_ = b_cnt; off_opts_ = b_cnt + b_done; off_rows_ = off_opts_ + b_opts; hoff_out_ = b_opts;
            cap_ = cap;
            bpo_ = bpo_cap;
        }
        char* d = dev_.template as<char>();
        v->d_cnt = reinterpret_cast<uint32_t*>(d);
        v->d_done = reinterpret_cast<uint32_t*>(d + off_done_);
        v->d_opts = reinterpret_cast<Opt*>(d + off_opts_);
        v->d_rows = reinterpret_cast<double*>(d + off_rows_);
        v->h_opts = host_.template as<Opt>();
        v->h_out = reinterpret_cast<const double*>(host_.template as<char>() + hoff_out_);
        v->d_out = reinterpret_cast<double*>(host_.template alias<char>() + hoff_out_);
        return 0;
    }
};

}

#ifdef __HIPCC__
#include <hip/hip_runtime.h>

namespace olmc {

int device_mem_fail(hipError_t e, const char* call);

struct HipMem {
    using Stream = hipStream_t;
    static int status(hipError_t e, const char* call) { return e == hipSuccess ? 0 : device_mem_fail(e, call); }
    static int alloc(void** p, size_t bytes) { return status(hipMalloc(p, bytes), "hipMalloc"); }
    static int free(void* p) { return status(hipFree(p), "hipFree"); }
    static int alloc_pinned(void** p, size_t bytes, bool mapped) {
        return status(hipHostMalloc(p, bytes, mapped ? hipHostMallocMapped : hipHostMallocDefault), "hipHostMalloc");
    }
    static int free_pinned(void* p) { return status(hipHostFree(p), "hipHostFree"); }
    static int device_alias(void** d, void* h) { return status(hipHostGetDevicePointer(d, h, 0), "hipHostGetDevicePointer"); }
    static int upload(void* d, const void* h, size_t bytes, Stream s) { return status(hipMemcpyAsync(d, h, bytes, hipMemcpyHostToDevice, s), "hipMemcpyAsync"); }
    static int zero(void* d, size_t bytes, Stream s) { return status(hipMemsetAsync(d, 0, bytes, s), "hipMemsetAsync"); }
    static int wait(Stream s) { return status(hipStreamSynchronize(s), "hipStreamSynchronize"); }
};

}
#endif

#endif
```

optionslab_amd/csrc/olmc_host_math.h:

```cpp
#ifndef OLMC_HOST_MATH_H
#define OLMC_HOST_MATH_H

#include "olmc.h"
#include "olmc_jump_scenarios.h"

#include <algorithm>
#include <cmath>
#include <cstdint>
#include <cstring>

namespace olmc {

struct Contract {
    double a;
    double vol;
    double strike;
    double sign;
    double scale;
    double neg_sign_strike;
    double sign_scale;
};

template <int NSETS>
struct ContractSet {
// ... 416 lines not shown
    std::stable_sort(order, order + k, [&](int32_t x, int32_t y) {
        return group[x] != group[y] ? group[x] < group[y] : spot_of[x] < spot_of[y];
    });
    for (int32_t j = 0; j < k; ++j) {
        const int32_t i = order[j];
        set->slot[j][kScnLogS] = log_s[i];
        set->slot[j][kScnMuDt] = mu_dt[i];
        set->slot[j][kScnStrike] = sc[i].K;
        set->slot[j][kScnSign] = sc[i].is_call ? 1.0 : -1.0;
        set->fresh[j] = j == 0 || group[order[j - 1]] != group[i] || spot_of[order[j - 1]] != spot_of[i];
        set->end[group[i]] = j + 1;
        slot_of[i] = j;
    }
    for (int32_t g = set->n_recursions; g < kHestonRecursions; ++g) set->end[g] = k;
    return nullptr;
}

inline void heston_greeks_scenarios(const GreeksSet& gs, double kappa, double theta, double sigma_v, double rho, olmc_heston_scenario* sc) {
    for (int i = 0; i < gs.k; ++i) {
        const olmc_option& o = gs.o[i];
        sc[i] = olmc_heston_scenario{o.S, o.K, o.T, o.r, o.q, kappa, theta, sigma_v, rho, o.sigma * o.sigma, o.is_call, 0};
    }
}

constexpr int kJumpGroups = OLMC_MAX_BATCH;

struct JumpScenarioSet {
    double grp[kJumpGroups][6];
    double slot[OLMC_MAX_BATCH][6];
    int32_t end[kJumpGroups];
    int32_t fresh[OLMC_MAX_BATCH];
    int32_t kou_mask;
    int32_t n_groups;
    double p0_floor;
};
enum { kJsP0, kJsLamDt, kJsC1, kJsC2, kJsC3 };
enum { kJsLogS, kJsVol, kJsNDrift, kJsStrike, kJsSign };

inline bool same_jump_group(const oljs_scenario& x, const oljs_scenario& y) {
    return x.model == y.model && same_bits(x.lambda_j, y.lambda_j) && same_bits(x.T, y.T) && same_bits(x.a1, y.a1) && same_bits(x.a2, y.a2)
        && (x.model == OLMC_JUMP_MERTON || same_bits(x.a3, y.a3));
}

inline const char* jump_scenario_groups(const oljs_scenario* sc, int32_t k, int32_t* n_groups, int32_t* group) {
    if (k < 1 || k > OLMC_MAX_BATCH) return "the number of scenarios must be in [1, OLMC_MAX_BATCH]";
    int32_t first[kJumpGroups], n = 0;
    for (int32_t i = 0; i < k; ++i) {
        int32_t g = 0;
        while (g < n && !same_jump_group(sc[first[g]], sc[i])) ++g;
        if (g == n) first[n++] = i;
        group[i] = g;
    }
    *n_groups = n;
    return nullptr;
}

inline bool jump_scenario_poisoned(const oljs_scenario& s) {
    return poisoned(s.S, s.K, s.T, s.r, s.sigma, s.q) || std::isnan(s.lambda_j + s.a1 + s.a2 + s.a3);
}

inline double jump_kappa(int model, double a1, double a2, double a3) {
    return model == OLMC_JUMP_MERTON ? std::exp(a1 + 0.5 * a2 * a2) - 1 : a1 * a2 / (a2 - 1) + (1 - a1) * a3 / (a3 + 1) - 1;
}

inline const char* jump_scenario_set(const oljs_scenario* sc, int32_t k, int32_t n_steps, JumpScenarioSet* set, int32_t* slot_of) {
    std::memset(set, 0, sizeof *set);
    int32_t group[OLMC_MAX_BATCH], spot_of[OLMC_MAX_BATCH], order[OLMC_MAX_BATCH];
    double log_s[OLMC_MAX_BATCH], vol[OLMC_MAX_BATCH], n_drift[OLMC_MAX_BATCH];
    if (const char* bad = jump_scenario_groups(sc, k, &set->n_groups, group)) return bad;
    set->p0_floor = 1.0;
    for (int32_t i = 0; i < k; ++i) {
        const oljs_scenario& s = sc[i];
        const double dt = s.T / n_steps;
        const int32_t g = group[i];
        const bool kou = s.model != OLMC_JUMP_MERTON;
        double* const cst = set->grp[g];
        cst[kJsLamDt] = s.lambda_j * dt;
        cst[kJsP0] = std::exp(-cst[kJsLamDt]);
        cst[kJsC1] = s.a1;
        cst[kJsC2] = kou ? 1.0 / s.a2 : s.a2;
        cst[kJsC3] = kou ? 1.0 / s.a3 : 0.0;
        if (kou) set->kou_mask |= 1 << g;
        set->p0_floor = cst[kJsP0] < set->p0_floor ? cst[kJsP0] : (std::isnan(cst[kJsP0]) ? 0.0 : set->p0_floor);
        const double drift = (s.r - s.q - s.lambda_j * jump_kappa(s.model, s.a1, s.a2, s.a3) - 0.5 * s.sigma * s.sigma) * dt;
        log_s[i] = std::log(s.S);
        vol[i] = s.sigma * std::sqrt(dt) * kZScale;
        n_drift[i] = static_cast<double>(n_steps) * drift;
        spot_of[i] = i;
        for (int32_t j = 0; j < i; ++j)
            if (group[j] == g && same_bits(log_s[j], log_s[i]) && same_bits(vol[j], vol[i]) && same_bits(n_drift[j], n_drift[i])) { spot_of[i] = spot_of[j]; break; }
        order[i] = i;
    }
    std::stable_sort(order, order + k, [&](int32_t x, int32_t y) {
        return group[x] != group[y] ? group[x] < group[y] : spot_of[x] < spot_of[y];
    });
    for (int32_t j = 0; j < k; ++j) {
        const int32_t i = order[j];
        set->slot[j][kJsLogS] = log_s[i];
        set->slot[j][kJsVol] = vol[i];
        set->slot[j][kJsNDrift] = n_drift[i];
        set->slot[j][kJsStrike] = sc[i].K;
        set->slot[j][kJsSign] = sc[i].is_call ? 1.0 : -1.0;
        set->fresh[j] = j == 0 || group[order[j - 1]] != group[i] || spot_of[order[j - 1]] != spot_of[i];
        set->end[group[i]] = j + 1;
        slot_of[i] = j;
    }
    for (int32_t g = set->n_groups; g < kJumpGroups; ++g) set->end[g] = k;
    return nullptr;
}

inline void jump_greeks_scenarios(const GreeksSet& gs, const oljd_model& m, oljs_scenario* sc) {
    for (int i = 0; i < gs.k; ++i) {
        const olmc_option& o = gs.o[i];
        sc[i] = oljs_scenario{o.S, o.K, o.T, o.r, o.sigma, o.q, o.is_call, m.model, m.lambda_j, m.a1, m.a2, m.a3};
    }
}

inline void shard_range(int64_t n_paths, int rank, int n_ranks, int64_t* lo, int64_t* count) {
    const int64_t a = n_paths * rank / n_ranks, b = n_paths * (rank + 1) / n_ranks;
    *lo = a;
    *count = b - a;
}

constexpr int64_t kQmcShardAlign = 512, kQmcShardMinPoints = 4096;
inline void qmc_shard_range(int64_t n_points, int rank, int n_ranks, int64_t* lo, int64_t* count) {
    if (n_points / n_ranks < kQmcShardMinPoints) return shard_range(n_points, rank, n_ranks, lo, count);
    const int64_t a = n_points * rank / n_ranks / kQmcShardAlign * kQmcShardAlign;
    const int64_t b = rank + 1 == n_ranks ? n_points : n_points * (rank + 1) / n_ranks / kQmcShardAlign * kQmcShardAlign;
    *lo = a;
    *count = b - a;
}

constexpr int kBlock = 256;
constexpr int kWave = 64;
constexpr int kWavesPerBlock = kBlock / kWave;
constexpr int kQmcBlock = 8;
constexpr int32_t kMaxGrid = 1 << 18;
constexpr int32_t kShortPathSteps = 128, kShortPathGrid = 4096;
constexpr int64_t kQmcPathMaxGrid = 8192;
constexpr size_t kHestonSlabCap = size_t(1) << 30;
constexpr int32_t kHestonBridgeBlocksPerCu = 2;

inline int32_t path_grid(int64_t n_paths, int32_t n_steps, int grid_cap) {
    int64_t cap = grid_cap > 0 ? std::min<int64_t>(grid_cap, kMaxGrid) : kMaxGrid;
    if (grid_cap == 0 && n_steps <= kShortPathSteps) cap = kShortPathGrid;
    return static_cast<int32_t>(std::min<int64_t>((n_paths + kBlock - 1) / kBlock, cap));
}

inline int32_t qmc_wave_grid(int64_t units, int grid_cap) {
    const int64_t cap = grid_cap > 0 ? std::min<int64_t>(grid_cap, kQmcPathMaxGrid) : kQmcPathMaxGrid;
    return static_cast<int32_t>(std::min<int64_t>((units + kWavesPerBlock - 1) / kWavesPerBlock, cap));
}
inline int32_t qmc_point_grid(int64_t n_points, int grid_cap) { return qmc_wave_grid(n_points, grid_cap); }
inline int32_t qmc_blocks_grid(int64_t blocks, int grid_cap) { return qmc_wave_grid(blocks, grid_cap); }

struct QmcShape {
    bool blocks, split, aligned, aligned8;
    int64_t units;
    int32_t grid;
};
inline QmcShape qmc_launch_shape(int64_t point_offset, int64_t n_paths, int32_t dims, int qmc_block, int grid_cap) {
    QmcShape sh;
    sh.aligned = (point_offset & 63) == 0 && dims >= 32;
    sh.aligned8 = (point_offset & 511) == 0;
    const int blocks_from_log2 = dims < 32 ? 19 : dims < 64 ? 20 : dims < 128 ? 21 : 22;
    sh.blocks = qmc_block == 1 ? true : (qmc_block != 0 ? false : n_paths >= (int64_t(1) << blocks_from_log2));
    const int64_t split_grid = (n_paths + kWave - 1) / kWave;
    sh.split = !sh.blocks && (qmc_block == 0 || qmc_block == 2) && dims >= 16 && split_grid <= kMaxGrid;
    sh.units = sh.blocks ? (point_offset + n_paths + kQmcBlock - 1) / kQmcBlock - point_offset / kQmcBlock : n_paths;
    sh.grid = sh.split ? static_cast<int32_t>(split_grid) : path_grid(sh.units, INT32_MAX, grid_cap);
    return sh;
}

struct HestonSlabs {
    size_t slab;
    int32_t fit;
    int32_t grid;
    size_t bytes;
};
inline HestonSlabs heston_slab_shape(int32_t n_steps, int32_t grid, int cus, int32_t factors = 2) {
    HestonSlabs s;
    s.slab = static_cast<size_t>(factors) * static_cast<size_t>(n_steps) * kWave * sizeof(double);
    s.fit = static_cast<int32_t>(std::max<size_t>(kHestonSlabCap / (s.slab * kWavesPerBlock), 1));
    s.grid = std::min(grid, std::min(s.fit, std::max(cus, 1) * kHestonBridgeBlocksPerCu));
    s.bytes = s.slab * kWavesPerBlock * static_cast<size_t>(s.grid);
    return s;
}

}

#endif
```

optionslab_amd/csrc/olmc_kernels.h:

```cpp
#pragma once
#include <type_traits>
#include <hip/hip_runtime.h>
#include <stdint.h>

#include "olmc_host_math.h"

namespace olmc {



struct Words4 {
    uint32_t x0, x1, x2, x3;
};

__device__ __forceinline__ uint32_t xor3(uint32_t a, uint32_t b, uint32_t c) {
    return __builtin_amdgcn_bitop3_b32(a, b, c, 0x96);
}

__device__ __forceinline__ Words4 philox4x32_10(uint32_t c0, uint32_t c1, uint32_t c2, uint32_t c3,
                                                uint32_t k0, uint32_t k1) {
#pragma unroll
    for (int round = 0; round < 10; ++round) {
        const uint64_t p0 = static_cast<uint64_t>(kPhiloxM0) * c0;
        const uint64_t p1 = static_cast<uint64_t>(kPhiloxM1) * c2;
// ... 2358 lines not shown
#pragma unroll
                        for (int b = 0; b < 9; ++b) lo[b] = next[b];
                    }
                    ndtri_lockstep_add<kQmcBlock>(q, u, z0);
                }
            }
        } else {
            for (int32_t t = t0; t < t1; ++t) {
                const uint32_t* __restrict__ row = sv + static_cast<size_t>(t) * kSobolBits;
                uint32_t x = shift[t];
                const int z0 = opaque_zero();
#pragma unroll
                for (int b = B0; b < kSobolBits; ++b) x = __builtin_amdgcn_bitop3_b32(x, row[b], mask[b], 0x78);
                double u[kQmcBlock];
#pragma unroll
                for (int p = 0; p < kQmcBlock; ++p) {
                    if (p) x ^= row[__builtin_ctz(static_cast<unsigned>(p))];
                    u[p] = sobol_uniform(x);
                }
                ndtri_lockstep_add<kQmcBlock>(q, u, z0);
            }
        }
#pragma unroll
        for (int p = 0; p < kQmcBlock; ++p) zs[p][threadIdx.x] += q[p];
    }
}

template <int MODE, bool ALIGNED = false >
__global__ __launch_bounds__(kBlock) __attribute__((amdgpu_waves_per_eu(ALIGNED ? 4 : 3, 8))) void european_qmc_block_kernel(QmcRange qr, Contract c, const uint32_t* __restrict__ sv,
                                                                    const uint32_t* __restrict__ shift, ReduceWs ws,
                                                                    double* __restrict__ terminal) {
    constexpr int NV = MODE == kControlVariate ? 5 : 2;
    double acc[NV] = {};
    const uint64_t base = qr.first / kQmcBlock;
    const uint64_t last = qr.first + static_cast<uint64_t>(qr.count);
    const int64_t n_blocks = static_cast<int64_t>((last + kQmcBlock - 1) / kQmcBlock - base);
    const int64_t stride = static_cast<int64_t>(gridDim.x) * kBlock;
    const int64_t lane = ALIGNED ? static_cast<int64_t>(threadIdx.x & (kWave - 1)) : 0;
    for (int64_t i = static_cast<int64_t>(blockIdx.x) * kBlock + threadIdx.x; i - lane < n_blocks; i += stride) {
        const uint64_t k0 = (base + static_cast<uint64_t>(i)) * kQmcBlock;
        const uint32_t gray = static_cast<uint32_t>(k0 ^ (k0 >> 1));
        uint32_t mask[kSobolBits];
#pragma unroll
        for (int b = 2; b < kSobolBits; ++b) mask[b] = 0u - ((gray >> b) & 1u);
        __shared__ double zs[kQmcBlock][kBlock];
        qmc_block_sums<2, ALIGNED>(mask, qr.dims, sv, shift, zs, ALIGNED ? static_cast<uint32_t>(__builtin_amdgcn_readfirstlane(static_cast<int>(gray))) : 0u);
#pragma unroll 1
        for (int p = 0; p < kQmcBlock; ++p) {
            const uint64_t k = k0 + static_cast<uint64_t>(p);
            if (k < qr.first || k >= last) continue;
            const double zp = zs[p][threadIdx.x];
            const double st = exp(c.a + c.vol * zp);
            if constexpr (MODE == kTerminal) {
                const int64_t at = static_cast<int64_t>(k - qr.first);
                terminal[at] = st;
                if (qr.mirror) terminal[qr.count + at] = exp(c.a - c.vol * zp);
            } else {
                add_sample<MODE>(acc, fmax(c.sign * (st - c.strike), 0.0), st);
            }
        }
    }
    if constexpr (MODE != kTerminal) block_then_grid_reduce<NV>(acc, ws);
}

template <int NSETS, bool BLOCK8, bool SPLIT = false, bool ALIGNED = false >
__global__ __launch_bounds__(kBlock) __attribute__((amdgpu_waves_per_eu((BLOCK8 && ALIGNED) ? 4 : 1, 8))) void european_qmc_batch_kernel(QmcRange qr, ContractSet<NSETS> cs, const uint32_t* __restrict__ sv,
                                                                    const uint32_t* __restrict__ shift, ReduceWs ws) {
    static_assert(!(BLOCK8 && SPLIT), "a thread either carries eight points or a quarter of one point's dimensions");
    static_assert(SPLIT || BLOCK8 || !ALIGNED, "the aligned forms exist for split workgroups and for blocks of eight");
    constexpr int NV = 2 * NSETS;
    double acc[NV];
    if constexpr (SPLIT) {
        __shared__ double quarter_sum[kWavesPerBlock][kWave];
        const int wave = __builtin_amdgcn_readfirstlane(static_cast<int>(threadIdx.x) / kWave), lane = threadIdx.x & (kWave - 1);
        const int64_t i = static_cast<int64_t>(blockIdx.x) * kWave + lane;
        const uint64_t k = qr.first + static_cast<uint64_t>((ALIGNED || i < qr.count) ? i : 0);
        const uint32_t gray = static_cast<uint32_t>(k ^ (k >> 1));
        uint32_t mask[kSobolBits];
#pragma unroll
        for (int b = 0; b < kSobolBits; ++b) mask[b] = 0u - ((gray >> b) & 1u);
        const uint32_t gray_hi = ALIGNED ? static_cast<uint32_t>(__builtin_amdgcn_readfirstlane(static_cast<int>(gray))) : 0u;
        {
            NdtriRegs regs;
            if constexpr (ALIGNED) regs.load();
            quarter_sum[wave][lane] = qmc_point_sum<ALIGNED>(mask, qmc_quarter_begin(qr.dims, wave), qmc_quarter_begin(qr.dims, wave + 1), sv, shift, gray_hi, &regs);
        }
        __syncthreads();
#pragma unroll
        for (int j = 0; j < NV; ++j) acc[j] = 0.0;
        if (wave == 0) {
            const double zsum = ((quarter_sum[0][lane] + quarter_sum[1][lane]) + quarter_sum[2][lane]) + quarter_sum[3][lane];
            european_payoffs<NSETS, false, kReduce>(cs, zsum, i < qr.count, 0, 0, nullptr, acc);
        }
    } else if constexpr (BLOCK8) {
        const int64_t i = static_cast<int64_t>(blockIdx.x) * kBlock + threadIdx.x;
        const uint64_t base = qr.first / kQmcBlock;
        const uint64_t last = qr.first + static_cast<uint64_t>(qr.count);
        const int64_t n_units = static_cast<int64_t>((last + kQmcBlock - 1) / kQmcBlock - base);
        const bool unit_live = i < n_units;
        const uint64_t k0 = (base + static_cast<uint64_t>((ALIGNED || unit_live) ? i : 0)) * kQmcBlock;
        const uint32_t gray = static_cast<uint32_t>(k0 ^ (k0 >> 1));
        uint32_t mask[kSobolBits];
#pragma unroll
        for (int b = 2; b < kSobolBits; ++b) mask[b] = 0u - ((gray >> b) & 1u);
        __shared__ double zs[kQmcBlock][kBlock];
        qmc_block_sums<2, ALIGNED>(mask, qr.dims, sv, shift, zs, ALIGNED ? static_cast<uint32_t>(__builtin_amdgcn_readfirstlane(static_cast<int>(gray))) : 0u);
#pragma unroll
        for (int j = 0; j < NV; ++j) acc[j] = 0.0;
        uint32_t live_points = 0u;
#pragma unroll
        for (int p = 0; p < kQmcBlock; ++p) {
            const uint64_t k = k0 + static_cast<uint64_t>(p);
            live_points |= (unit_live && k >= qr.first && k < last) ? (1u << p) : 0u;
        }
#pragma unroll 1
        for (int p = 0; p < kQmcBlock; ++p)
            european_payoffs<NSETS, false, kReduce>(cs, zs[p][threadIdx.x], ((live_points >> p) & 1u) != 0u, 0, 0, nullptr, acc);
    } else {
        const int64_t i = static_cast<int64_t>(blockIdx.x) * kBlock + threadIdx.x;
        const bool live = i < qr.count;
        const uint64_t k = qr.first + static_cast<uint64_t>(live ? i : 0);
        const uint32_t gray = static_cast<uint32_t>(k ^ (k >> 1));
        uint32_t mask[kSobolBits];
#pragma unroll
        for (int b = 0; b < kSobolBits; ++b) mask[b] = 0u - ((gray >> b) & 1u);
        double zsum = 0.0;
#pragma unroll 1
        for (int w = 0; w < 4; ++w) zsum += qmc_point_sum(mask, qmc_quarter_begin(qr.dims, w), qmc_quarter_begin(qr.dims, w + 1), sv, shift);
#pragma unroll
        for (int j = 0; j < NV; ++j) acc[j] = 0.0;
        european_payoffs<NSETS, false, kReduce>(cs, zsum, live, 0, 0, nullptr, acc);
    }
    block_then_grid_reduce<NV>(acc, ws);
}

__global__ void publish_kernel(const double* __restrict__ src, int32_t n, double* __restrict__ host_dst, uint64_t* __restrict__ done_flag,
                               uint64_t done_value) {
    if (static_cast<int32_t>(threadIdx.x) < n) host_dst[threadIdx.x] = src[threadIdx.x];
    __builtin_amdgcn_fence(__ATOMIC_RELEASE, "");
    if (threadIdx.x == 0) __hip_atomic_store(done_flag, done_value, __ATOMIC_RELAXED, __HIP_MEMORY_SCOPE_SYSTEM);
}

constexpr int kQmcBridgeMaxSteps = 1024;
enum QmcPathFamily { kQmcAsianArithmetic = 0, kQmcAsianGeometric = 1, kQmcExtrema = 2,
                     kPathEuropean = 3 };

struct QmcBridgePlan {
    const uint32_t* ab;
    const double* coef;
};

__device__ __forceinline__ void wave_lds_sync() { asm volatile("s_waitcnt lgkmcnt(0)" ::: "memory"); }

__device__ __forceinline__ double qmc_normal(const uint32_t* __restrict__ sv, const uint32_t* __restrict__ shift, int32_t t, uint32_t gray) {
    const uint32_t* __restrict__ row = sv + static_cast<size_t>(t) * kSobolBits;
    uint32_t x = shift[t];
    for (uint32_t g = gray; g != 0u; g &= g - 1u) x ^= row[__builtin_ctz(g)];
    return ndtri_w_add(0.0, sobol_uniform(x), opaque_zero());
}

__device__ __forceinline__ double wave_allsum(double v) {
#pragma unroll
    for (int off = 1; off < kWave; off <<= 1) v += __shfl_xor(v, off, kWave);
    return v;
}
__device__ __forceinline__ double wave_allmax(double v) {
#pragma unroll
    for (int off = 1; off < kWave; off <<= 1) v = max_f64(v, __shfl_xor(v, off, kWave));
    return v;
}
__device__ __forceinline__ double wave_allmin(double v) {
#pragma unroll
    for (int off = 1; off < kWave; off <<= 1) v = min_f64(v, __shfl_xor(v, off, kWave));
    return v;
}

struct QmcLeg {
    double a = 0.0, mx = 0.0, mn = 0.0;
};

template <int FAMILY>
__device__ __forceinline__ void qmc_leg_add(QmcLeg& g, double y ) {
    if constexpr (FAMILY == kQmcAsianArithmetic) g.a += exp2_f64(y);
    else if constexpr (FAMILY == kQmcAsianGeometric) g.a += y;
    else { g.mx = max_f64(g.mx, y); g.mn = min_f64(g.mn, y); }
}

template <int FAMILY>
__device__ __forceinline__ double qmc_payoff(const ExtremaContract& c, double inv_steps, double a, double mx, double mn, double y_n) {
    if constexpr (FAMILY == kQmcExtrema) return extrema_payoff(c, y_n, mx, mn);
    const double avg = FAMILY == kQmcAsianArithmetic ? c.s0 * (a * inv_steps) : c.s0 * exp(a * inv_steps);
    return fmax(c.sign * (avg - c.strike), 0.0);
}

template <int FAMILY>
__device__ __forceinline__ double qmc_leg_payoff(const ExtremaContract& c, double inv_steps, const QmcLeg& g, double y_n) {
    if constexpr (FAMILY == kQmcExtrema) return qmc_payoff<FAMILY>(c, inv_steps, 0.0, wave_allmax(g.mx), wave_allmin(g.mn), y_n);
    return qmc_payoff<FAMILY>(c, inv_steps, wave_allsum(g.a), 0.0, 0.0, y_n);
}

__device__ __forceinline__ void qmc_bridge_fill(const uint32_t* __restrict__ sv, const uint32_t* __restrict__ shift, const QmcBridgePlan& plan,
                                                double* W, int32_t n, int lane, uint32_t gray) {
    wave_lds_sync();
    for (int32_t c0 = 0; c0 < n; c0 += kWave) {
        const int32_t node = c0 + lane;
        const bool live = node < n;
        const double z = qmc_normal(sv, shift, live ? node : n - 1, gray);
        uint32_t ab = 0u;
        double ca = 0.0, cb = 0.0, sd = 0.0;
        if (live && node > 0) {
            ab = plan.ab[node];
            ca = plan.coef[node]; cb = plan.coef[n + node]; sd = plan.coef[2 * n + node];
        }
        const int32_t a = static_cast<int32_t>(ab & 0xffffu), b = static_cast<int32_t>(ab >> 16), m = (a + b) >> 1;
        if (c0 == 0) {
            if (lane == 0) { W[0] = 0.0; W[n] = sqrt(static_cast<double>(n)) * z; }
            wave_lds_sync();
#pragma unroll 1
            for (int lvl = 0; lvl < 6 && (1 << lvl) < n; ++lvl) {
                if (live && node >= (1 << lvl) && node < (2 << lvl)) W[m] = __builtin_fma(ca, W[a], __builtin_fma(cb, W[b], sd * z));
                wave_lds_sync();
            }
        } else {
            if (live) W[m] = __builtin_fma(ca, W[a], __builtin_fma(cb, W[b], sd * z));
            wave_lds_sync();
        }
    }
}

template <bool BRIDGE, typename Body>
__device__ __forceinline__ double qmc_point_walk(const uint32_t* __restrict__ sv, const uint32_t* __restrict__ shift, const QmcBridgePlan& plan,
                                                 double* W, int32_t n, int lane, uint32_t gray, Body body) {
    if constexpr (BRIDGE) {
        qmc_bridge_fill(sv, shift, plan, W, n, lane, gray);
        for (int32_t c0 = 0; c0 < n; c0 += kWave) {
            const int32_t j = c0 + lane + 1;
            if (j <= n) body(j, W[j]);
        }
        return W[n];
    } else {
        double carry = 0.0;
        for (int32_t c0 = 0; c0 < n; c0 += kWave) {
            const int32_t t = c0 + lane;
            double s = t < n ? qmc_normal(sv, shift, t, gray) : 0.0;
#pragma unroll
            for (int off = 1; off < kWave; off <<= 1) {
                const double o = __shfl_up(s, off, kWave);
                if (lane >= off) s += o;
            }
            const double wj = carry + s;
            carry += __shfl(s, kWave - 1, kWave);
            if (t < n) body(t + 1, wj);
        }
        return carry;
    }
}

template <int FAMILY, bool BRIDGE, bool ANTI>
__global__ __launch_bounds__(kBlock) void qmc_path_kernel(QmcRange qr, ExtremaContract c, double inv_steps, const uint32_t* __restrict__ sv,
                                                          const uint32_t* __restrict__ shift, QmcBridgePlan plan, ReduceWs ws) {
    constexpr double kLog2e = 1.4426950408889634;
    constexpr double kUnit = FAMILY == kQmcAsianArithmetic ? kLog2e : 1.0;
    const int lane = static_cast<int>(threadIdx.x) & (kWave - 1);
    const int wave = __builtin_amdgcn_readfirstlane(static_cast<int>(threadIdx.x) / kWave);
    const int32_t n = qr.dims;
    const double drift = c.drift * kUnit, vol = c.vol * kUnit;
    double acc[2] = {0.0, 0.0};
    [[maybe_unused]] double* W = nullptr;
    if constexpr (BRIDGE) {
        __shared__ double w_lds[kWavesPerBlock][kQmcBridgeMaxSteps + 1];
        W = w_lds[wave];
    }
    const int64_t stride = static_cast<int64_t>(gridDim.x) * kWavesPerBlock;
    for (int64_t i = static_cast<int64_t>(blockIdx.x) * kWavesPerBlock + wave; i < qr.count; i += stride) {
        const uint64_t k = qr.first + static_cast<uint64_t>(i);
        const uint32_t gray = static_cast<uint32_t>(__builtin_amdgcn_readfirstlane(static_cast<int>(k ^ (k >> 1))));
        QmcLeg up, dn;
        const double w_n = qmc_point_walk<BRIDGE>(sv, shift, plan, W, n, lane, gray, [&](int32_t j, double wj) {
            const double jd = static_cast<double>(j) * drift;
            qmc_leg_add<FAMILY>(up, __builtin_fma(vol, wj, jd));
            if constexpr (ANTI) qmc_leg_add<FAMILY>(dn, __builtin_fma(-vol, wj, jd));
        });
        const double nd = static_cast<double>(n) * c.drift;
        const double xu = qmc_leg_payoff<FAMILY>(c, inv_steps, up, __builtin_fma(c.vol, w_n, nd));
        if (lane == 0) { acc[0] += xu; acc[1] += xu * xu; }
        if constexpr (ANTI) {
            const double xd = qmc_leg_payoff<FAMILY>(c, inv_steps, dn, __builtin_fma(-c.vol, w_n, nd));
            if (lane == 0) { acc[0] += xd; acc[1] += xd * xd; }
        }
    }
    block_then_grid_reduce<2>(acc, ws);
}

__device__ __forceinline__ uint32_t qmc_date_quotient(int32_t j, uint32_t magic) { return __umulhi(2u * static_cast<uint32_t>(j), magic); }

__device__ __forceinline__ int32_t wave_allmin_i32(int32_t v) {
#pragma unroll
    for (int off = 1; off < kWave; off <<= 1) v = min(v, __shfl_xor(v, off, kWave));
    return v;
}

__device__ __forceinline__ double qmc_autocall_payoff(const AutocallContract& c, double obs_rate, int32_t first, double mn, double y_n) {
    if (first <= c.n_obs) {
        const double k = static_cast<double>(first);
        return (1.0 + c.coupon_unit * k) * exp(obs_rate * k);
    }
    double fin = 1.0;
    if (y_n >= c.log_coupon) fin += c.final_coupon;
    if (mn <= c.log_ki && y_n < 0.0) fin = exp(y_n);
    return fin * c.final_df;
}

template <bool BRIDGE, bool ANTI>
__global__ __launch_bounds__(kBlock) void qmc_autocall_kernel(QmcRange qr, AutocallContract c, double obs_rate, uint32_t obs_magic,
                                                              const uint32_t* __restrict__ sv, const uint32_t* __restrict__ shift,
                                                              QmcBridgePlan plan, ReduceWs ws) {
    constexpr int LEGS = ANTI ? 2 : 1;
    constexpr int32_t kNever = 0x7fffffff;
    const int lane = static_cast<int>(threadIdx.x) & (kWave - 1);
    const int wave = __builtin_amdgcn_readfirstlane(static_cast<int>(threadIdx.x) / kWave);
    const int32_t n = qr.dims;
    const uint32_t f = static_cast<uint32_t>(c.obs_freq);
    double acc[2] = {0.0, 0.0};
    [[maybe_unused]] double* W = nullptr;
    if constexpr (BRIDGE) {
        __shared__ double w_lds[kWavesPerBlock][kQmcBridgeMaxSteps + 1];
        W = w_lds[wave];
    }
    const int64_t stride = static_cast<int64_t>(gridDim.x) * kWavesPerBlock;
    for (int64_t i = static_cast<int64_t>(blockIdx.x) * kWavesPerBlock + wave; i < qr.count; i += stride) {
        const uint64_t k = qr.first + static_cast<uint64_t>(i);
        const uint32_t gray = static_cast<uint32_t>(__builtin_amdgcn_readfirstlane(static_cast<int>(k ^ (k >> 1))));
        double mn[LEGS];
        int32_t first[LEGS];
#pragma unroll
        for (int leg = 0; leg < LEGS; ++leg) { mn[leg] = 0.0; first[leg] = kNever; }
        const double w_n = qmc_point_walk<BRIDGE>(sv, shift, plan, W, n, lane, gray, [&](int32_t j, double wj) {
            const double jd = static_cast<double>(j) * c.drift;
            const uint32_t obs = qmc_date_quotient(j, obs_magic);
            const bool observed = obs * f == static_cast<uint32_t>(j);
#pragma unroll
            for (int leg = 0; leg < LEGS; ++leg) {
                const double y = __builtin_fma(leg ? -c.vol : c.vol, wj, jd);
                mn[leg] = min_f64(mn[leg], y);
                first[leg] = (observed && y >= c.log_autocall) ? min(first[leg], static_cast<int32_t>(obs)) : first[leg];
            }
        });
        const double nd = static_cast<double>(n) * c.drift;
#pragma unroll
        for (int leg = 0; leg < LEGS; ++leg) {
            const double x = qmc_autocall_payoff(c, obs_rate, wave_allmin_i32(first[leg]), wave_allmin(mn[leg]),
                                                 __builtin_fma(leg ? -c.vol : c.vol, w_n, nd));
            if (lane == 0) { acc[0] += x; acc[1] += x * x; }
        }
    }
    block_then_grid_reduce<2>(acc, ws);
}

template <bool BRIDGE, bool ANTI>
__global__ __launch_bounds__(kBlock) void qmc_cliquet_kernel(QmcRange qr, CliquetContract c, uint32_t period_magic,
                                                             const uint32_t* __restrict__ sv, const uint32_t* __restrict__ shift,
                                                             QmcBridgePlan plan, ReduceWs ws) {
    constexpr int LEGS = ANTI ? 2 : 1;
    const int lane = static_cast<int>(threadIdx.x) & (kWave - 1);
    const int wave = __builtin_amdgcn_readfirstlane(static_cast<int>(threadIdx.x) / kWave);
    const int32_t n = qr.dims, spp = c.steps_per_period;
    [[maybe_unused]] const int32_t used = spp * c.n_periods;
    const double period_drift = spp * c.drift;
    double acc[2] = {0.0, 0.0};
    [[maybe_unused]] double* W = nullptr;
    if constexpr (BRIDGE) {
        __shared__ double w_lds[kWavesPerBlock][kQmcBridgeMaxSteps + 1];
        W = w_lds[wave];
    }
    const int64_t stride = static_cast<int64_t>(gridDim.x) * kWavesPerBlock;
    for (int64_t i = static_cast<int64_t>(blockIdx.x) * kWavesPerBlock + wave; i < qr.count; i += stride) {
        const uint64_t k = qr.first + static_cast<uint64_t>(i);
        const uint32_t gray = static_cast<uint32_t>(__builtin_amdgcn_readfirstlane(static_cast<int>(k ^ (k >> 1))));
        double total[LEGS];
#pragma unroll
        for (int leg = 0; leg < LEGS; ++leg) total[leg] = 0.0;
        auto add_period = [&](double dw ) {
#pragma unroll
            for (int leg = 0; leg < LEGS; ++leg) {
                const double local = exp(__builtin_fma(leg ? -c.vol : c.vol, dw, period_drift)) - 1.0;
                total[leg] += fmin(fmax(local, c.local_floor), c.local_cap);
            }
        };
        if constexpr (BRIDGE) {
            qmc_bridge_fill(sv, shift, plan, W, n, lane, gray);
            for (int32_t p0 = 0; p0 < c.n_periods; p0 += kWave) {
                const int32_t p = p0 + lane;
                if (p < c.n_periods) add_period(W[(p + 1) * spp] - W[p * spp]);
            }
        } else {
            double w_reset = 0.0;
            qmc_point_walk<false>(sv, shift, plan, W, used, lane, gray, [&](int32_t j, double wj) {
                const int32_t c0 = __builtin_amdgcn_readfirstlane(j - lane - 1);
                const double w_before = __shfl_up(wj, static_cast<unsigned int>(spp), kWave);
                const double w_start = lane >= spp ? w_before : w_reset;
                if (qmc_date_quotient(j, period_magic) * static_cast<uint32_t>(spp) == static_cast<uint32_t>(j)) add_period(wj - w_start);
                const int32_t last = static_cast<int32_t>(qmc_date_quotient(min(c0 + kWave, used), period_magic)) * spp;
                if (last > c0) w_reset = __shfl(wj, last - c0 - 1, kWave);
            });
        }
#pragma unroll
        for (int leg = 0; leg < LEGS; ++leg) {
            const double clipped = fmin(fmax(wave_allsum(total[leg]), c.global_floor), c.global_cap);
            const double x = fmax(clipped, 0.0) * c.s0;
            if (lane == 0) { acc[0] += x; acc[1] += x * x; }
        }
    }
    block_then_grid_reduce<2>(acc, ws);
}

template <int FAMILY, bool BRIDGE, bool ANTI, int NSETS>
__global__ __launch_bounds__(kBlock) void qmc_path_greeks_kernel(QmcRange qr, ExtremaGreeksSet gs, double inv_steps, const uint32_t* __restrict__ sv,
                                                                 const uint32_t* __restrict__ shift, QmcBridgePlan plan, ReduceWs ws) {
    constexpr double kLog2e = 1.4426950408889634;
    constexpr double kUnit = FAMILY == kQmcAsianArithmetic ? kLog2e : 1.0;
    constexpr int G = kAsianGroups, LEGS = ANTI ? 2 : 1, NV = 2 * NSETS;
    constexpr int P = pow2_ceil(LEGS * G), SHIFT = 6 - log2_of(P);
    static_assert(NSETS <= kWave, "one lane per contract");
    const int lane = static_cast<int>(threadIdx.x) & (kWave - 1);
    const int wave = __builtin_amdgcn_readfirstlane(static_cast<int>(threadIdx.x) / kWave);
    const int32_t n = qr.dims;
    double drift[G], vol[G];
#pragma unroll
    for (int g = 0; g < G; ++g) { drift[g] = gs.drift[g] * kUnit; vol[g] = gs.vol[g] * kUnit; }
    const int s = lane < NSETS ? lane : 0;
    int32_t grp = gs.group[0];
#pragma unroll
    for (int k = 1; k < NSETS; ++k) {
        const int32_t gk = gs.group[k];
        grp = s == k ? gk : grp;
    }
    ExtremaContract c;
    c.s0 = pick_recursion(s, gs.s0);
    c.log_barrier_rel = pick_recursion(s, gs.log_barrier_rel);
    c.drift = pick_recursion(grp, gs.drift);
    c.vol = pick_recursion(grp, gs.vol);
    c.strike = gs.strike;
    c.sign = gs.sign;
    c.payoff = gs.payoff;
    c.pad = 0;
    const int src_up = grp << SHIFT, src_dn = (G + grp) << SHIFT;
    double acc[2] = {0.0, 0.0};
    [[maybe_unused]] double* W = nullptr;
    if constexpr (BRIDGE) {
        __shared__ double w_lds[kWavesPerBlock][kQmcBridgeMaxSteps + 1];
        W = w_lds[wave];
    }
    const int64_t stride = static_cast<int64_t>(gridDim.x) * kWavesPerBlock;
    for (int64_t i = static_cast<int64_t>(blockIdx.x) * kWavesPerBlock + wave; i < qr.count; i += stride) {
        const uint64_t k = qr.first + static_cast<uint64_t>(i);
        const uint32_t gray = static_cast<uint32_t>(__builtin_amdgcn_readfirstlane(static_cast<int>(k ^ (k >> 1))));
        QmcLeg leg[LEGS][G];
        const double w_n = qmc_point_walk<BRIDGE>(sv, shift, plan, W, n, lane, gray, [&](int32_t j, double wj) {
            const double jj = static_cast<double>(j);
#pragma unroll
            for (int g = 0; g < G; ++g) {
                const double jd = jj * drift[g];
                qmc_leg_add<FAMILY>(leg[0][g], __builtin_fma(vol[g], wj, jd));
                if constexpr (ANTI) qmc_leg_add<FAMILY>(leg[1][g], __builtin_fma(-vol[g], wj, jd));
            }
        });
        double a_up = 0.0, a_dn = 0.0, mx_up = 0.0, mx_dn = 0.0, mn_up = 0.0, mn_dn = 0.0;
        if constexpr (FAMILY == kQmcExtrema) {
            double vmx[P], vmn[P];
#pragma unroll
            for (int v = 0; v < P; ++v) {
                vmx[v] = v < LEGS * G ? leg[v / G][v % G].mx : 0.0;
                vmn[v] = v < LEGS * G ? leg[v / G][v % G].mn : 0.0;
            }
            wave_transpose_reduce<P, kWave / 2, MaxOp>(vmx);
            wave_transpose_reduce<P, kWave / 2, MinOp>(vmn);
            mx_up = __shfl(vmx[0], src_up, kWave);
            mn_up = __shfl(vmn[0], src_up, kWave);
            if constexpr (ANTI) { mx_dn = __shfl(vmx[0], src_dn, kWave); mn_dn = __shfl(vmn[0], src_dn, kWave); }
        } else {
            double va[P];
#pragma unroll
            for (int v = 0; v < P; ++v) va[v] = v < LEGS * G ? leg[v / G][v % G].a : 0.0;
            wave_transpose_reduce<P>(va);
            a_up = __shfl(va[0], src_up, kWave);
            if constexpr (ANTI) a_dn = __shfl(va[0], src_dn, kWave);
        }
        const double nd = static_cast<double>(n) * c.drift;
        const double xu = qmc_payoff<FAMILY>(c, inv_steps, a_up, mx_up, mn_up, __builtin_fma(c.vol, w_n, nd));
        acc[0] += xu; acc[1] += xu * xu;
        if constexpr (ANTI) {
            const double xd = qmc_payoff<FAMILY>(c, inv_steps, a_dn, mx_dn, mn_dn, __builtin_fma(-c.vol, w_n, nd));
            acc[0] += xd; acc[1] += xd * xd;
        }
    }
    __shared__ double stage[kWavesPerBlock][NV];
    if (lane < NSETS) { stage[wave][2 * lane] = acc[0]; stage[wave][2 * lane + 1] = acc[1]; }
    __syncthreads();
    double row = 0.0;
    if (threadIdx.x < NV) {
        row = stage[0][threadIdx.x];
#pragma unroll
        for (int w = 1; w < kWavesPerBlock; ++w) row += stage[w][threadIdx.x];
    }
    grid_reduce_workgroup<NV>(row, ws);
}

template <bool BRIDGE, bool PATH_MAJOR>
__global__ __launch_bounds__(kBlock) void lsm_qmc_paths_kernel(QmcRange qr, LsmContract c, const uint32_t* __restrict__ sv,
                                                               const uint32_t* __restrict__ shift, QmcBridgePlan plan, double* paths) {
    const int lane = static_cast<int>(threadIdx.x) & (kWave - 1);
    const int32_t n = qr.dims;
    const int64_t count = qr.count;
    const int64_t n_blocks = (count + kWave - 1) / kWave;
    const int64_t stride = static_cast<int64_t>(gridDim.x) * kWavesPerBlock;
    const int wave = __builtin_amdgcn_readfirstlane(static_cast<int>(threadIdx.x) / kWave);
    for (int64_t blk = static_cast<int64_t>(blockIdx.x) * kWavesPerBlock + wave; blk < n_blocks; blk += stride) {
        const int64_t i = blk * kWave + lane;
        const bool live = i < count;
        const uint32_t k = static_cast<uint32_t>(i);
        const uint32_t gray = k ^ (k >> 1);
        const uint32_t gray_hi = static_cast<uint32_t>(__builtin_amdgcn_readfirstlane(static_cast<int>(gray))) & ~63u;
        uint32_t mask[6];
#pragma unroll
        for (int b = 0; b < 6; ++b) mask[b] = 0u - ((gray >> b) & 1u);
        auto at = [&](int32_t t) { return path_at<PATH_MAJOR>(i, t, count, n); };
        if (live) paths[at(0)] = c.s_first;
        double w = 0.0;
        for (int32_t c0 = 0; c0 < n; c0 += kWave) {
            const int32_t tl = c0 + lane < n ? c0 + lane : n - 1;
            const uint32_t* __restrict__ mine = sv + static_cast<size_t>(tl) * kSobolBits;
            uint32_t fold = shift[tl];
#pragma unroll
            for (int b = 6; b < kSobolBits; ++b) fold ^= mine[b] & (0u - ((gray_hi >> b) & 1u));
            const int32_t cn = n - c0 < kWave ? n - c0 : kWave;
            for (int32_t d = 0; d < cn; ++d) {
                const int32_t t = c0 + d;
                const uint32_t* __restrict__ row = sv + static_cast<size_t>(t) * kSobolBits;
                uint32_t x = static_cast<uint32_t>(__shfl(static_cast<int>(fold), d, kWave));
#pragma unroll
                for (int b = 0; b < 6; ++b) x = __builtin_amdgcn_bitop3_b32(x, row[b], mask[b], 0x78);
                const double z = ndtri_w_add(0.0, sobol_uniform(x), opaque_zero());
                if constexpr (BRIDGE) {
                    if (t == 0) {
                        if (live) paths[at(n)] = sqrt(static_cast<double>(n)) * z;
                    } else {
                        const uint32_t ab = plan.ab[t];
                        const int32_t a = static_cast<int32_t>(ab & 0xffffu), b = static_cast<int32_t>(ab >> 16), m = (a + b) >> 1;
                        const double ca = plan.coef[t], cb = plan.coef[n + t], sd = plan.coef[2 * n + t];
                        if (live) {
                            const double wa = a == 0 ? 0.0 : paths[at(a)];
                            paths[at(m)] = __builtin_fma(ca, wa, __builtin_fma(cb, paths[at(b)], sd * z));
                        }
                    }
                } else {
                    w += z;
                    if (live) paths[at(t + 1)] = exp(c.log_s0 + __builtin_fma(c.vol, w, static_cast<double>(t + 1) * c.drift));
                }
            }
        }
        if constexpr (BRIDGE) {
            if (live) {
                for (int32_t j = 1; j <= n; ++j) {
                    const size_t p = at(j);
                    paths[p] = exp(c.log_s0 + __builtin_fma(c.vol, paths[p], static_cast<double>(j) * c.drift));
                }
            }
        }
    }
}

constexpr int kHestonQmcBatch = 4;

struct QmcLanePoint {
    uint32_t gray_hi;
    uint32_t mask[6];
    __device__ __forceinline__ explicit QmcLanePoint(uint32_t k ) {
        const uint32_t gray = k ^ (k >> 1);
        gray_hi = static_cast<uint32_t>(__builtin_amdgcn_readfirstlane(static_cast<int>(gray))) & ~63u;
#pragma unroll
        for (int b = 0; b < 6; ++b) mask[b] = 0u - ((gray >> b) & 1u);
    }
};

template <bool EVEN_NORMAL, typename Body>
__device__ __forceinline__ void heston_qmc_draws(const uint32_t* __restrict__ sv, const uint32_t* __restrict__ shift, int32_t n, int lane,
                                                 const QmcLanePoint& lp, Body body) {
    const int32_t dims = 2 * n;
    for (int32_t c0 = 0; c0 < dims; c0 += kWave) {
        const int32_t tl = c0 + lane < dims ? c0 + lane : dims - 1;
        const uint32_t* __restrict__ mine = sv + static_cast<size_t>(tl) * kSobolBits;
        uint32_t fold = shift[tl];
#pragma unroll
        for (int b = 6; b < kSobolBits; ++b) fold ^= mine[b] & (0u - ((lp.gray_hi >> b) & 1u));
        const int32_t cn = dims - c0 < kWave ? dims - c0 : kWave;
        for (int32_t d = 0; d < cn; d += 2) {
            double p[2];
#pragma unroll
            for (int h = 0; h < 2; ++h) {
                const uint32_t* __restrict__ row = sv + static_cast<size_t>(c0 + d + h) * kSobolBits;
                uint32_t x = static_cast<uint32_t>(__shfl(static_cast<int>(fold), d + h, kWave));
#pragma unroll
                for (int b = 0; b < 6; ++b) x = __builtin_amdgcn_bitop3_b32(x, row[b], lp.mask[b], 0x78);
                p[h] = sobol_uniform(x);
                if (EVEN_NORMAL || h == 1) p[h] = ndtri_w_add(0.0, p[h], opaque_zero());
            }
            body((c0 + d) >> 1, p[0], p[1]);
        }
    }
}

template <typename At>
__device__ __forceinline__ void heston_qmc_bridge_fill(const uint32_t* __restrict__ sv, const uint32_t* __restrict__ shift, const QmcBridgePlan& plan,
                                                       int32_t n, int lane, const QmcLanePoint& lp, bool live, double* w1, double* w2, At at) {
    heston_qmc_draws<true>(sv, shift, n, lane, lp, [&](int32_t k, double z1, double z2) {
        if (k == 0) {
            const double sq = sqrt(static_cast<double>(n));
            if (live) { w1[at(n)] = sq * z1; w2[at(n)] = sq * z2; }
        } else {
            const uint32_t ab = plan.ab[k];
            const int32_t a = static_cast<int32_t>(ab & 0xffffu), b = static_cast<int32_t>(ab >> 16), m = (a + b) >> 1;
            const double ca = plan.coef[k], cb = plan.coef[n + k], sd = plan.coef[2 * n + k];
            if (live) {
                const double a1 = a == 0 ? 0.0 : w1[at(a)], a2 = a == 0 ? 0.0 : w2[at(a)];
                const double b1 = w1[at(b)], b2 = w2[at(b)];
                w1[at(m)] = __builtin_fma(ca, a1, __builtin_fma(cb, b1, sd * z1));
                w2[at(m)] = __builtin_fma(ca, a2, __builtin_fma(cb, b2, sd * z2));
            }
        }
    });
}

template <typename At, typename Step>
__device__ __forceinline__ void heston_qmc_bridge_sweep(int32_t n, const double* w1, const double* w2, At at, Step step) {
    double p1 = 0.0, p2 = 0.0;
    for (int32_t t0 = 0; t0 < n; t0 += kHestonQmcBatch) {
        double q1[kHestonQmcBatch], q2[kHestonQmcBatch];
#pragma unroll
        for (int j = 0; j < kHestonQmcBatch; ++j) {
            const int32_t jj = t0 + j + 1 <= n ? t0 + j + 1 : n;
            q1[j] = w1[at(jj)];
            q2[j] = w2[at(jj)];
        }
#pragma unroll
        for (int j = 0; j < kHestonQmcBatch; ++j) {
            if (t0 + j < n) {
                step(t0 + j, q1[j] - p1, q2[j] - p2);
                p1 = q1[j]; p2 = q2[j];
// ... 952 lines not shown
```

Before: 2514 billion.

## Walk consecutive Sobol points incrementally via Gray-code state kept in LDS

Each wave now handles a run of consecutive QMC points. The first point of a run is built from the full Gray-code XOR over direction numbers, and each later point takes one XOR with a transposed direction-vector column, with the per-dimension state kept in dynamic LDS. This replaces the per-point popcount-length XOR loop with a single lookup, at the cost of LDS state, fewer waves in the grid, and extra host work to build the transposed table. It applies only to the QMC path, autocall, cliquet and greeks kernels, not the Philox GBM European benchmark.

Result: no change. 2494 billion (-0.8%).

```diff
diff --git a/include/olmc.h b/include/olmc.h
--- a/include/olmc.h
+++ b/include/olmc.h
@@ -315,7 +315,7 @@
 
 int olmc_profile_enable(int on);
 enum { OLMC_TUNE_GRID_CAP = 2, OLMC_TUNE_QMC_BLOCK = 4, OLMC_TUNE_SPLIT_TAIL = 7, OLMC_TUNE_POLL = 8, OLMC_TUNE_SPLIT_SAT = 9,
-       OLMC_TUNE_MULTI_LAUNCH = 10, OLMC_TUNE_STAGED_COPY = 11, OLMC_TUNE_PHILOX_TABLE = 12 };
+       OLMC_TUNE_MULTI_LAUNCH = 10, OLMC_TUNE_STAGED_COPY = 11, OLMC_TUNE_PHILOX_TABLE = 12, OLMC_TUNE_QMC_RUN = 13 };
 int olmc_tune(int knob, int value);
 int olmc_profile_reset(void);
 int olmc_kernel_time(int64_t* launches, double* total_ms);
diff --git a/optionslab_amd/_hip.py b/optionslab_amd/_hip.py
--- a/optionslab_amd/_hip.py
+++ b/optionslab_amd/_hip.py
@@ -1040,6 +1040,7 @@
 TUNE_MULTI_LAUNCH = 10
 TUNE_STAGED_COPY = 11
 TUNE_PHILOX_TABLE = 12
+TUNE_QMC_RUN = 13
 
 
 def tune(knob: int, value: int) -> None:
diff --git a/optionslab_amd/csrc/olmc.hip b/optionslab_amd/csrc/olmc.hip
--- a/optionslab_amd/csrc/olmc.hip
+++ b/optionslab_amd/csrc/olmc.hip
@@ -334,6 +334,7 @@
 
 int g_multi_launch = 0;
 int g_grid_cap = 0;
+int g_qmc_run = 0;
 int g_qmc_block = 0;
 int g_poll = 0;
 int g_split_tail = 0;
@@ -535,6 +536,13 @@
 void launch_timed(Kernel kernel, dim3 grid, dim3 block, hipStream_t s, const EventPair* timed, const Args&... args) {
     if (timed) hipExtLaunchKernelGGL(kernel, grid, block, 0, s, timed->start, timed->stop, 0, args...);
     else hipLaunchKernelGGL(kernel, grid, block, 0, s, args...);
+}
+
+template <typename Kernel, typename... Args>
+void launch_qmc_runs(Kernel kernel, int32_t grid, hipStream_t s, const EventPair* timed, const QmcRange& qr, const QmcRuns& rn, const Args&... args) {
+    const uint32_t lds = rn.run > 1 ? static_cast<uint32_t>(sizeof(uint32_t)) * kWavesPerBlock * qr.dims : 0u;
+    if (timed) hipExtLaunchKernelGGL(kernel, dim3(grid), dim3(kBlock), lds, s, timed->start, timed->stop, 0, args...);
+    else hipLaunchKernelGGL(kernel, dim3(grid), dim3(kBlock), lds, s, args...);
 }
 
 template <typename F>
@@ -1731,12 +1739,18 @@
     }
 };
 
-int qmc_table(DeviceCtx* c, const SobolCall& q, const uint32_t** d_sv, const uint32_t** d_shift) {
-    const size_t sv_words = static_cast<size_t>(q.dims()) * kSobolBits;
-    const int rc = c->sobol.put(q.sv, sizeof(uint32_t) * sv_words, q.shift, sizeof(uint32_t) * q.dims(), c->stream, [c] { return c->drain(); });
+int qmc_table(DeviceCtx* c, const SobolCall& q, const uint32_t** d_sv, const uint32_t** d_shift, const uint32_t** d_sv_t = nullptr) {
+    const size_t dims = static_cast<size_t>(q.dims()), sv_words = dims * kSobolBits;
+    const int rc = c->sobol.put_derived(q.sv, sizeof(uint32_t) * sv_words, q.shift, sizeof(uint32_t) * dims, sizeof(uint32_t) * sv_words,
+                                        [dims](unsigned char* dst, const unsigned char* sv, const unsigned char*) {
+                                            for (size_t t = 0; t < dims; ++t)
+                                                for (size_t b = 0; b < kSobolBits; ++b)
+                                                    std::memcpy(dst + sizeof(uint32_t) * (b * dims + t), sv + sizeof(uint32_t) * (t * kSobolBits + b), sizeof(uint32_t));
+                                        }, c->stream, [c] { return c->drain(); });
     if (rc) return rc;
     *d_sv = c->sobol.device<uint32_t>();
     *d_shift = *d_sv + sv_words;
+    if (d_sv_t) *d_sv_t = *d_shift + dims;
     return OLMC_OK;
 }
 
@@ -1889,13 +1903,14 @@
     const uint32_t* d_shift;
     QmcBridgePlan plan;
     QmcRange qr;
+    QmcRuns runs;
     int32_t grid;
     bool bridge, anti;
     double inv_steps;
     double* slabs = nullptr;
 };
 int qmc_path_setup(DeviceCtx* c, const SobolCall& q, QmcPathLaunch* pl) {
-    int rc = qmc_table(c, q, &pl->d_sv, &pl->d_shift);
+    int rc = qmc_table(c, q, &pl->d_sv, &pl->d_shift, &pl->runs.sv_t);
     if (rc) return rc;
     pl->plan = QmcBridgePlan{nullptr, nullptr};
     pl->bridge = q.bridge;
@@ -1904,7 +1919,8 @@
         if (rc) return rc;
     }
     pl->qr = q.range();
-    pl->grid = qmc_point_grid(q.count, g_grid_cap);
+    pl->runs.run = qmc_run_length(q.count, q.dims(), g_qmc_run);
+    pl->grid = qmc_run_grid(q.count, pl->runs.run, g_grid_cap);
     pl->anti = q.anti;
     pl->inv_steps = 1.0 / q.n_steps;
     return OLMC_OK;
@@ -1954,7 +1970,7 @@
     return run_qmc_reduce(*q, 2, qmc_point_shape, [&](int32_t g, hipStream_t s, const EventPair* timed, const QmcPathLaunch& pl, const ReduceWs& ws) {
         with_qmc_path_family(family, [&](auto f) {
             with_bridge_anti(pl, [&](auto b, auto a) {
-                launch_timed(qmc_path_kernel<f, b, a>, dim3(g), dim3(kBlock), s, timed, pl.qr, ec, pl.inv_steps, pl.d_sv, pl.d_shift, pl.plan, ws);
+                launch_qmc_runs(qmc_path_kernel<f, b, a>, g, s, timed, pl.qr, pl.runs, pl.qr, ec, pl.inv_steps, pl.d_sv, pl.d_shift, pl.runs, pl.plan, ws);
             });
         });
     }, qmc_stats(o.r, o.T, bad, out));
@@ -1975,8 +1991,8 @@
         with_qmc_path_family(family, [&](auto f) {
             with_bool(pl.bridge, [&](auto b) {
                 with_set_anti(nsets, pl.anti, [&](auto width, auto a) {
-                    launch_timed(qmc_path_greeks_kernel<f, b, a, width>, dim3(g), dim3(kBlock), s, timed, pl.qr, es, pl.inv_steps, pl.d_sv, pl.d_shift,
-                                 pl.plan, ws);
+                    launch_qmc_runs(qmc_path_greeks_kernel<f, b, a, width>, g, s, timed, pl.qr, pl.runs, pl.qr, es, pl.inv_steps, pl.d_sv, pl.d_shift,
+                                    pl.runs, pl.plan, ws);
                 });
             });
         });
@@ -2041,7 +2057,7 @@
     const uint32_t magic = qmc_date_magic(observation_freq);
     return run_qmc_reduce(*call, 2, qmc_point_shape, [&](int32_t g, hipStream_t s, const EventPair* timed, const QmcPathLaunch& pl, const ReduceWs& ws) {
         with_bridge_anti(pl, [&](auto b, auto m) {
-            launch_timed(qmc_autocall_kernel<b, m>, dim3(g), dim3(kBlock), s, timed, pl.qr, a.ac, a.obs_rate, magic, pl.d_sv, pl.d_shift, pl.plan, ws);
+            launch_qmc_runs(qmc_autocall_kernel<b, m>, g, s, timed, pl.qr, pl.runs, pl.qr, a.ac, a.obs_rate, magic, pl.d_sv, pl.d_shift, pl.runs, pl.plan, ws);
         });
     }, qmc_stats(0.0, T, a.bad, out));
 }
@@ -2060,7 +2076,7 @@
     const bool bad = cliquet_poisoned(S, T, r, sigma, q, local_cap, local_floor, global_cap, global_floor);
     return run_qmc_reduce(*call, 2, qmc_point_shape, [&](int32_t g, hipStream_t s, const EventPair* timed, const QmcPathLaunch& pl, const ReduceWs& ws) {
         with_bridge_anti(pl, [&](auto b, auto m) {
-            launch_timed(qmc_cliquet_kernel<b, m>, dim3(g), dim3(kBlock), s, timed, pl.qr, cc, magic, pl.d_sv, pl.d_shift, pl.plan, ws);
+            launch_qmc_runs(qmc_cliquet_kernel<b, m>, g, s, timed, pl.qr, pl.runs, pl.qr, cc, magic, pl.d_sv, pl.d_shift, pl.runs, pl.plan, ws);
         });
     }, qmc_stats(r, T, bad, out));
 }
@@ -3898,6 +3914,7 @@
 extern "C" int olmc_tune(int knob, int value) {
     if (knob == OLMC_TUNE_GRID_CAP && value >= 0) { g_grid_cap = value; return OLMC_OK; }
     if (knob == OLMC_TUNE_QMC_BLOCK && value >= -1 && value <= 2) { g_qmc_block = value; return OLMC_OK; }
+    if (knob == OLMC_TUNE_QMC_RUN && value >= 0 && value <= kQmcRunKnobMax) { g_qmc_run = value; return OLMC_OK; }
     if (knob == OLMC_TUNE_POLL && value >= -1 && value <= 0) { g_poll = value; return OLMC_OK; }
     if (knob == OLMC_TUNE_SPLIT_TAIL && value >= -1 && value <= 0) { g_split_tail = value; return OLMC_OK; }
     if (knob == OLMC_TUNE_SPLIT_SAT && value >= 0 && value <= 16) { g_split_sat = value; return OLMC_OK; }
diff --git a/optionslab_amd/csrc/olmc_device_mem.h b/optionslab_amd/csrc/olmc_device_mem.h
--- a/optionslab_amd/csrc/olmc_device_mem.h
+++ b/optionslab_amd/csrc/olmc_device_mem.h
@@ -105,6 +105,16 @@
     int put(const void* a, size_t na, const void* b, size_t nb, typename B::Stream s, Quiesce&& quiesce) {
         if (valid_ && mirror_.size() == na + nb && std::memcmp(mirror_.data(), a, na) == 0 && std::memcmp(mirror_.data() + na, b, nb) == 0) return 0;
         return refill(na + nb, s, quiesce, [&](unsigned char* m) { std::memcpy(m, a, na); std::memcpy(m + na, b, nb); return 0; });
+    }
+    template <typename Quiesce, typename Derive>
+    int put_derived(const void* a, size_t na, const void* b, size_t nb, size_t nd, Derive&& derive, typename B::Stream s, Quiesce&& quiesce) {
+        if (valid_ && mirror_.size() == na + nb + nd && std::memcmp(mirror_.data(), a, na) == 0 && std::memcmp(mirror_.data() + na, b, nb) == 0) return 0;
+        return refill(na + nb + nd, s, quiesce, [&](unsigned char* m) {
+            std::memcpy(m, a, na);
+            std::memcpy(m + na, b, nb);
+            derive(m + na + nb, m, m + na);
+            return 0;
+        });
     }
     template <typename Quiesce, typename Build>
     int ensure(int64_t key, size_t bytes, typename B::Stream s, Quiesce&& quiesce, Build&& build) {
diff --git a/optionslab_amd/csrc/olmc_host_math.h b/optionslab_amd/csrc/olmc_host_math.h
--- a/optionslab_amd/csrc/olmc_host_math.h
+++ b/optionslab_amd/csrc/olmc_host_math.h
@@ -592,6 +592,17 @@
     return static_cast<int32_t>(std::min<int64_t>((units + kWavesPerBlock - 1) / kWavesPerBlock, cap));
 }
 inline int32_t qmc_point_grid(int64_t n_points, int grid_cap) { return qmc_wave_grid(n_points, grid_cap); }
+
+constexpr int32_t kQmcRunMaxDims = 1024, kQmcRunMax = 16, kQmcRunKnobMax = 1024;
+constexpr int64_t kQmcRunMinRuns = 4096;
+inline int32_t qmc_run_length(int64_t n_points, int32_t dims, int qmc_run) {
+    if (dims > kQmcRunMaxDims) return 1;
+    if (qmc_run > 0) return std::min(qmc_run, kQmcRunKnobMax);
+    int32_t run = 1;
+    while (run < kQmcRunMax && n_points / (2 * run) >= kQmcRunMinRuns) run *= 2;
+    return run;
+}
+inline int32_t qmc_run_grid(int64_t n_points, int32_t run, int grid_cap) { return qmc_wave_grid((n_points + run - 1) / run, grid_cap); }
 inline int32_t qmc_blocks_grid(int64_t blocks, int grid_cap) { return qmc_wave_grid(blocks, grid_cap); }
 
 struct QmcShape {
diff --git a/optionslab_amd/csrc/olmc_kernels.h b/optionslab_amd/csrc/olmc_kernels.h
--- a/optionslab_amd/csrc/olmc_kernels.h
+++ b/optionslab_amd/csrc/olmc_kernels.h
@@ -2534,10 +2534,49 @@
 
 __device__ __forceinline__ void wave_lds_sync() { asm volatile("s_waitcnt lgkmcnt(0)" ::: "memory"); }
 
-__device__ __forceinline__ double qmc_normal(const uint32_t* __restrict__ sv, const uint32_t* __restrict__ shift, int32_t t, uint32_t gray) {
-    const uint32_t* __restrict__ row = sv + static_cast<size_t>(t) * kSobolBits;
-    uint32_t x = shift[t];
-    for (uint32_t g = gray; g != 0u; g &= g - 1u) x ^= row[__builtin_ctz(g)];
+struct QmcRuns {
+    const uint32_t* sv_t;
+    int32_t run;
+};
+
+struct QmcPoint {
+    uint32_t gray;
+    const uint32_t* step;
+    uint32_t* state;
+    bool keep;
+};
+
+template <typename Body>
+__device__ __forceinline__ void qmc_run_points(const QmcRange& qr, const QmcRuns& rn, int wave, Body body) {
+    extern __shared__ uint32_t qmc_state_lds[];
+    const int64_t run = rn.run;
+    const int64_t stride = static_cast<int64_t>(gridDim.x) * kWavesPerBlock * run;
+    QmcPoint p;
+    p.keep = rn.run > 1;
+    p.state = qmc_state_lds + (p.keep ? wave * qr.dims : 0);
+    for (int64_t lo = (static_cast<int64_t>(blockIdx.x) * kWavesPerBlock + wave) * run; lo < qr.count; lo += stride) {
+        const int64_t hi = lo + run < qr.count ? lo + run : qr.count;
+        for (int64_t i = lo; i < hi; ++i) {
+            const uint64_t k = qr.first + static_cast<uint64_t>(i);
+            p.gray = static_cast<uint32_t>(__builtin_amdgcn_readfirstlane(static_cast<int>(k ^ (k >> 1))));
+            const int col = __builtin_amdgcn_readfirstlane(i > lo ? __builtin_ctz(static_cast<uint32_t>(k)) : 0);
+            p.step = i > lo ? rn.sv_t + static_cast<size_t>(col) * qr.dims : nullptr;
+            body(p);
+        }
+    }
+}
+
+__device__ __forceinline__ double qmc_normal(const uint32_t* __restrict__ sv, const uint32_t* __restrict__ shift, int32_t t, const QmcPoint& p,
+                                             bool own = true) {
+    uint32_t x;
+    if (p.step) {
+        x = p.state[t] ^ p.step[t];
+    } else {
+        const uint32_t* __restrict__ row = sv + static_cast<size_t>(t) * kSobolBits;
+        x = shift[t];
+        for (uint32_t g = p.gray; g != 0u; g &= g - 1u) x ^= row[__builtin_ctz(g)];
+    }
+    if (p.keep && own) p.state[t] = x;
     return ndtri_w_add(0.0, sobol_uniform(x), opaque_zero());
 }
 
@@ -2582,12 +2621,12 @@
 }
 
 __device__ __forceinline__ void qmc_bridge_fill(const uint32_t* __restrict__ sv, const uint32_t* __restrict__ shift, const QmcBridgePlan& plan,
-                                                double* W, int32_t n, int lane, uint32_t gray) {
+                                                double* W, int32_t n, int lane, const QmcPoint& p) {
     wave_lds_sync();
     for (int32_t c0 = 0; c0 < n; c0 += kWave) {
         const int32_t node = c0 + lane;
         const bool live = node < n;
-        const double z = qmc_normal(sv, shift, live ? node : n - 1, gray);
+        const double z = qmc_normal(sv, shift, live ? node : n - 1, p, live);
         uint32_t ab = 0u;
         double ca = 0.0, cb = 0.0, sd = 0.0;
         if (live && node > 0) {
@@ -2612,9 +2651,9 @@
 
 template <bool BRIDGE, typename Body>
 __device__ __forceinline__ double qmc_point_walk(const uint32_t* __restrict__ sv, const uint32_t* __restrict__ shift, const QmcBridgePlan& plan,
-                                                 double* W, int32_t n, int lane, uint32_t gray, Body body) {
+                                                 double* W, int32_t n, int lane, const QmcPoint& p, Body body) {
     if constexpr (BRIDGE) {
-        qmc_bridge_fill(sv, shift, plan, W, n, lane, gray);
+        qmc_bridge_fill(sv, shift, plan, W, n, lane, p);
         for (int32_t c0 = 0; c0 < n; c0 += kWave) {
             const int32_t j = c0 + lane + 1;
             if (j <= n) body(j, W[j]);
@@ -2624,7 +2663,7 @@
         double carry = 0.0;
         for (int32_t c0 = 0; c0 < n; c0 += kWave) {
             const int32_t t = c0 + lane;
-            double s = t < n ? qmc_normal(sv, shift, t, gray) : 0.0;
+            double s = t < n ? qmc_normal(sv, shift, t, p) : 0.0;
 #pragma unroll
             for (int off = 1; off < kWave; off <<= 1) {
                 const double o = __shfl_up(s, off, kWave);
@@ -2640,7 +2679,7 @@
 
 template <int FAMILY, bool BRIDGE, bool ANTI>
 __global__ __launch_bounds__(kBlock) void qmc_path_kernel(QmcRange qr, ExtremaContract c, double inv_steps, const uint32_t* __restrict__ sv,
-                                                          const uint32_t* __restrict__ shift, QmcBridgePlan plan, ReduceWs ws) {
+                                                          const uint32_t* __restrict__ shift, QmcRuns rn, QmcBridgePlan plan, ReduceWs ws) {
     constexpr double kLog2e = 1.4426950408889634;
     constexpr double kUnit = FAMILY == kQmcAsianArithmetic ? kLog2e : 1.0;
     const int lane = static_cast<int>(threadIdx.x) & (kWave - 1);
@@ -2653,12 +2692,9 @@
         __shared__ double w_lds[kWavesPerBlock][kQmcBridgeMaxSteps + 1];
         W = w_lds[wave];
     }
-    const int64_t stride = static_cast<int64_t>(gridDim.x) * kWavesPerBlock;
-    for (int64_t i = static_cast<int64_t>(blockIdx.x) * kWavesPerBlock + wave; i < qr.count; i += stride) {
-        const uint64_t k = qr.first + static_cast<uint64_t>(i);
-        const uint32_t gray = static_cast<uint32_t>(__builtin_amdgcn_readfirstlane(static_cast<int>(k ^ (k >> 1))));
+    qmc_run_points(qr, rn, wave, [&](const QmcPoint& p) {
         QmcLeg up, dn;
-        const double w_n = qmc_point_walk<BRIDGE>(sv, shift, plan, W, n, lane, gray, [&](int32_t j, double wj) {
+        const double w_n = qmc_point_walk<BRIDGE>(sv, shift, plan, W, n, lane, p, [&](int32_t j, double wj) {
             const double jd = static_cast<double>(j) * drift;
             qmc_leg_add<FAMILY>(up, __builtin_fma(vol, wj, jd));
             if constexpr (ANTI) qmc_leg_add<FAMILY>(dn, __builtin_fma(-vol, wj, jd));
@@ -2670,7 +2706,7 @@
             const double xd = qmc_leg_payoff<FAMILY>(c, inv_steps, dn, __builtin_fma(-c.vol, w_n, nd));
             if (lane == 0) { acc[0] += xd; acc[1] += xd * xd; }
         }
-    }
+    });
     block_then_grid_reduce<2>(acc, ws);
 }
 
@@ -2696,7 +2732,7 @@
 template <bool BRIDGE, bool ANTI>
 __global__ __launch_bounds__(kBlock) void qmc_autocall_kernel(QmcRange qr, AutocallContract c, double obs_rate, uint32_t obs_magic,
                                                               const uint32_t* __restrict__ sv, const uint32_t* __restrict__ shift,
-                                                              QmcBridgePlan plan, ReduceWs ws) {
+                                                              QmcRuns rn, QmcBridgePlan plan, ReduceWs ws) {
     constexpr int LEGS = ANTI ? 2 : 1;
     constexpr int32_t kNever = 0x7fffffff;
     const int lane = static_cast<int>(threadIdx.x) & (kWave - 1);
@@ -2709,15 +2745,12 @@
         __shared__ double w_lds[kWavesPerBlock][kQmcBridgeMaxSteps + 1];
         W = w_lds[wave];
     }
-    const int64_t stride = static_cast<int64_t>(gridDim.x) * kWavesPerBlock;
-    for (int64_t i = static_cast<int64_t>(blockIdx.x) * kWavesPerBlock + wave; i < qr.count; i += stride) {
-        const uint64_t k = qr.first + static_cast<uint64_t>(i);
-        const uint32_t gray = static_cast<uint32_t>(__builtin_amdgcn_readfirstlane(static_cast<int>(k ^ (k >> 1))));
+    qmc_run_points(qr, rn, wave, [&](const QmcPoint& p) {
         double mn[LEGS];
         int32_t first[LEGS];
 #pragma unroll
         for (int leg = 0; leg < LEGS; ++leg) { mn[leg] = 0.0; first[leg] = kNever; }
-        const double w_n = qmc_point_walk<BRIDGE>(sv, shift, plan, W, n, lane, gray, [&](int32_t j, double wj) {
+        const double w_n = qmc_point_walk<BRIDGE>(sv, shift, plan, W, n, lane, p, [&](int32_t j, double wj) {
             const double jd = static_cast<double>(j) * c.drift;
             const uint32_t obs = qmc_date_quotient(j, obs_magic);
             const bool observed = obs * f == static_cast<uint32_t>(j);
@@ -2735,14 +2768,14 @@
                                                  __builtin_fma(leg ? -c.vol : c.vol, w_n, nd));
             if (lane == 0) { acc[0] += x; acc[1] += x * x; }
         }
-    }
+    });
     block_then_grid_reduce<2>(acc, ws);
 }
 
 template <bool BRIDGE, bool ANTI>
 __global__ __launch_bounds__(kBlock) void qmc_cliquet_kernel(QmcRange qr, CliquetContract c, uint32_t period_magic,
                                                              const uint32_t* __restrict__ sv, const uint32_t* __restrict__ shift,
-                                                             QmcBridgePlan plan, ReduceWs ws) {
+                                                             QmcRuns rn, QmcBridgePlan plan, ReduceWs ws) {
     constexpr int LEGS = ANTI ? 2 : 1;
     const int lane = static_cast<int>(threadIdx.x) & (kWave - 1);
     const int wave = __builtin_amdgcn_readfirstlane(static_cast<int>(threadIdx.x) / kWave);
@@ -2755,10 +2788,7 @@
         __shared__ double w_lds[kWavesPerBlock][kQmcBridgeMaxSteps + 1];
         W = w_lds[wave];
     }
-    const int64_t stride = static_cast<int64_t>(gridDim.x) * kWavesPerBlock;
-    for (int64_t i = static_cast<int64_t>(blockIdx.x) * kWavesPerBlock + wave; i < qr.count; i += stride) {
-        const uint64_t k = qr.first + static_cast<uint64_t>(i);
-        const uint32_t gray = static_cast<uint32_t>(__builtin_amdgcn_readfirstlane(static_cast<int>(k ^ (k >> 1))));
+    qmc_run_points(qr, rn, wave, [&](const QmcPoint& p) {
         double total[LEGS];
 #pragma unroll
         for (int leg = 0; leg < LEGS; ++leg) total[leg] = 0.0;
@@ -2770,14 +2800,14 @@
             }
         };
         if constexpr (BRIDGE) {
-            qmc_bridge_fill(sv, shift, plan, W, n, lane, gray);
+            qmc_bridge_fill(sv, shift, plan, W, n, lane, p);
             for (int32_t p0 = 0; p0 < c.n_periods; p0 += kWave) {
                 const int32_t p = p0 + lane;
                 if (p < c.n_periods) add_period(W[(p + 1) * spp] - W[p * spp]);
             }
         } else {
             double w_reset = 0.0;
-            qmc_point_walk<false>(sv, shift, plan, W, used, lane, gray, [&](int32_t j, double wj) {
+            qmc_point_walk<false>(sv, shift, plan, W, used, lane, p, [&](int32_t j, double wj) {
                 const int32_t c0 = __builtin_amdgcn_readfirstlane(j - lane - 1);
                 const double w_before = __shfl_up(wj, static_cast<unsigned int>(spp), kWave);
                 const double w_start = lane >= spp ? w_before : w_reset;
@@ -2792,13 +2822,13 @@
             const double x = fmax(clipped, 0.0) * c.s0;
             if (lane == 0) { acc[0] += x; acc[1] += x * x; }
         }
-    }
+    });
     block_then_grid_reduce<2>(acc, ws);
 }
 
 template <int FAMILY, bool BRIDGE, bool ANTI, int NSETS>
 __global__ __launch_bounds__(kBlock) void qmc_path_greeks_kernel(QmcRange qr, ExtremaGreeksSet gs, double inv_steps, const uint32_t* __restrict__ sv,
-                                                                 const uint32_t* __restrict__ shift, QmcBridgePlan plan, ReduceWs ws) {
+                                                                 const uint32_t* __restrict__ shift, QmcRuns rn, QmcBridgePlan plan, ReduceWs ws) {
     constexpr double kLog2e = 1.4426950408889634;
     constexpr double kUnit = FAMILY == kQmcAsianArithmetic ? kLog2e : 1.0;
     constexpr int G = kAsianGroups, LEGS = ANTI ? 2 : 1, NV = 2 * NSETS;
@@ -2833,12 +2863,9 @@
         __shared__ double w_lds[kWavesPerBlock][kQmcBridgeMaxSteps + 1];
         W = w_lds[wave];
     }
-    const int64_t stride = static_cast<int64_t>(gridDim.x) * kWavesPerBlock;
-    for (int64_t i = static_cast<int64_t>(blockIdx.x) * kWavesPerBlock + wave; i < qr.count; i += stride) {
-        const uint64_t k = qr.first + static_cast<uint64_t>(i);
-        const uint32_t gray = static_cast<uint32_t>(__builtin_amdgcn_readfirstlane(static_cast<int>(k ^ (k >> 1))));
+    qmc_run_points(qr, rn, wave, [&](const QmcPoint& p) {
         QmcLeg leg[LEGS][G];
-        const double w_n = qmc_point_walk<BRIDGE>(sv, shift, plan, W, n, lane, gray, [&](int32_t j, double wj) {
+        const double w_n = qmc_point_walk<BRIDGE>(sv, shift, plan, W, n, lane, p, [&](int32_t j, double wj) {
             const double jj = static_cast<double>(j);
 #pragma unroll
             for (int g = 0; g < G; ++g) {
@@ -2875,7 +2902,7 @@
             const double xd = qmc_payoff<FAMILY>(c, inv_steps, a_dn, mx_dn, mn_dn, __builtin_fma(-c.vol, w_n, nd));
             acc[0] += xd; acc[1] += xd * xd;
         }
-    }
+    });
     __shared__ double stage[kWavesPerBlock][NV];
     if (lane < NSETS) { stage[wave][2 * lane] = acc[0]; stage[wave][2 * lane + 1] = acc[1]; }
     __syncthreads();
```
